# Mario5Gray/Stable-Diffusion-1.5-LCM-ONNX-RKNN2

Hardware: AMD Instinct MI355X
Metric: 512x512 4-step LCM images/sec (higher is better)
Workload: dtype f16; 1 GPU; SD1.5 LCM 512x512, 4 steps, guidance 1.0 (no CFG), batch 1 per GPU, fp16 (fp32 accumulate), hipGraph replay; seeded synthetic SD1.5-architecture weights; batch_per_gpu=1, global_batch=1, image=512x512, lcm_steps=4, parallelism=independent requests x1 (RCCL broadcast of prompt embeddings only)

## Files before the change

include/lcm_hip.h:

```cpp
#ifndef LCM_HIP_H
#define LCM_HIP_H
#include <stdint.h>
#ifdef __cplusplus
extern "C" {
#endif

#define LCM_OK 0
#define LCM_EINVAL (-1)
#define LCM_ENODEV (-2)
#define LCM_EUNSUPPORTED (-3)

#define LCM_EPI_NONE 0
#define LCM_EPI_GEGLU 1
#define LCM_EPI_QUICK_GELU 2
#define LCM_EPI_GELU 3

const char* lcm_last_error(void);
int lcm_version(void);
int lcm_device_info(int dev, char* arch_buf, int buf_len, int* cu_count, uint64_t* hbm_bytes);

int lcm_gemm_f16(const void* A, int lda, const void* A2, int lda2, int K1,
                 const void* W, const void* bias, const void* rowadd, int ld_rowadd, int rows_per_batch,
                 const void* res, int ldr, void* out, int ldo,
                 int M, int N, int K, int epilogue, float out_scale,
                 int batch, int64_t strideA, int64_t strideW, int64_t strideO, int img_rows,
                 void* stats_out, int64_t stats_bytes, int* slabs_per_image, void* stream);
int64_t lcm_stats_bytes(int M, int N, int img_rows);

int lcm_set_workspace(void* ptr, int64_t bytes);
int lcm_set_stream_workspace(void* stream, void* ptr, int64_t bytes);
int lcm_stream_create(void** stream_out);
int lcm_stream_destroy(void* stream);

int lcm_set_tuning(int target_wgs, int max_splits, int min_wgs);
int lcm_set_split_policy(int max_rows_per_image, int max_parts);
int lcm_set_seg_mode(int mode);

int lcm_plan_set(int kind, int M, int N, int K, int aux, int bm, int bn, int splits, int variant);
int lcm_plan_clear(void);
int lcm_canonical_splits(int kind, int m_img, int N, int K, int aux, int ph);

int lcm_gemm_ln_f16(const void* A, int lda, const void* W, const void* ln_g, const void* ln_c, float eps,
                    void* out, int ldo, int M, int N, int K, int epilogue, int img_rows, void* stream);

int lcm_mlp_geglu_f16(const void* x, int ldx, const void* W1, const void* ln_g, const void* ln_c, float eps,
                      const void* W2, const void* b2, void* out, int ldo, int M, int C, int img_rows, void* stream);
int lcm_ln_fold_refresh(const void* W, int N, int K, const void* c_base, const void* c_delta, float alpha,
                        void* g_out, void* c_out, void* stream);

int lcm_set_persist_n(int on);

int lcm_set_kernel_variant(int variant);

int lcm_gemm_tile_config(int M, int N, int batch);

int lcm_conv3x3_f16(const void* in, const void* W, const void* bias,
                    const void* rowadd, int ld_rowadd, const void* res, void* out,
                    int B, int Hin, int Win, int Cin, int Cout, int stride, int ups,
                    void* stats_out, int64_t stats_bytes, int* slabs_per_image, void* stream);

int lcm_conv3x3_down_f16(const void* in, const void* W, const void* bias, void* out, int B, int Hin, int Win, int Cin, int Cout,
                         void* stats_out, int64_t stats_bytes, int* slabs_per_image, void* stream);

int lcm_conv3x3_gn_f16(const void* in, int C1, const void* in2, int C2, const void* gn_scale, const void* gn_shift,
                       int silu, const void* W, const void* bias, const void* rowadd, int ld_rowadd, const void* res,
                       void* out, int B, int Hin, int Win, int Cout, int ups, void* stats_out, int64_t stats_bytes,
                       int* slabs_per_image, void* stream);
int lcm_groupnorm_affine_f16(const void* x, int C1, const void* x2, int C2, const void* gamma, const void* beta,
                             void* scale_out, void* shift_out, int B, int HW, int groups, float eps, void* ws,
                             void* stream);
int lcm_set_halo_pipe_threshold(int wgs);
int lcm_set_halo_prefetch(int on);
int lcm_set_staged_epilogue(int on);
int lcm_set_conv_impl(int impl);

int lcm_conv3x3_c4_f32in(const void* in, const void* pre_w, const void* pre_b, float in_scale,
                         const void* W, const void* bias, void* out, int B, int H, int Wd, int Cout, void* stream);

int lcm_conv3x3_c4_res_f32in(const void* in, const void* W, const void* bias, const void* res, void* out, int B, int H,
                             int Wd, int Cout, void* stream);

int lcm_hint_conv_u8(const void* in, const void* W, const void* bias, void* out, int B, int H, int Wd, int Cout, int silu,
                     void* stream);
int lcm_hint_conv_f16(const void* in, const void* W, const void* bias, void* out, int B, int H, int Wd, int Cin, int Cout,
                      int stride, int silu, void* stream);

int lcm_conv3x3_smalln(const void* in, const void* W, const void* bias, void* out, void* out_f32,
                       int B, int H, int Wd, int Cin, int Cout, int mode, void* stream);
int lcm_conv3x3_smalln_gn(const void* in, const void* gn_scale, const void* gn_shift, int silu, const void* W,
                          const void* bias, void* out, void* out_f32, int B, int H, int Wd, int Cin, int Cout,
                          int mode, void* stream);

int64_t lcm_groupnorm_ws_bytes(int B, int HW, int C, int groups);
int lcm_groupnorm_f16(const void* x, int C1, const void* x2, int C2, const void* gamma, const void* beta,
                      void* out, int B, int HW, int groups, float eps, int silu, void* ws, void* stream);

int lcm_set_gn_fused_bytes(int64_t bytes);
int lcm_groupnorm_from_stats_f16(const void* x, int C1, const void* x2, int C2, const void* stats1, int P1,
                                 const void* stats2, int P2, const void* gamma, const void* beta, void* out,
                                 int B, int HW, int groups, float eps, int silu, void* ws, void* stream);

int lcm_layernorm_f16(const void* x, const void* gamma, const void* beta, void* out, int M, int C, float eps,
                      void* stream);

int lcm_attention_f16(const void* Q, int ldq, const void* K, int ldk, const void* V, int ldv, void* out, int ldo,
                      int B, int heads, int Sq, int Sk, int d, float scale, int causal, void* stream);
int lcm_set_attention_waves(int waves);
int lcm_set_attention_impl(int impl);
int lcm_set_attention_ksplit(int on);

int lcm_embed_tokens_f16(const void* ids, const void* tok_emb, const void* pos_emb, void* out, int B, int S, int D,
                         int vocab, void* stream);

int lcm_prompt_emphasis_f16(const void* z, const void* w, void* out, int ldo, int n_chunks, int S, int D, void* stream);

int lcm_softmax_rows_f16(void* x, int rows, int n, int ld, void* stream);
int lcm_transpose_f16(const void* in, int ldi, void* out, int ldo, int R, int C, int batch,
                      int64_t stride_in, int64_t stride_out, void* stream);

int lcm_linear_smallm_f16(const void* x, int ldx, const void* W, const void* bias, const void* res, int ldr,
                          void* out, int ldo, int M, int N, int K, int silu_in, int silu_out, void* stream);
int lcm_linear_rows_f16(const void* x, int ldx, int x_rows, const void* W, const void* bias, const void* res, int ldr,
                        int res_rows, void* out, int ldo, int M, int N, int K, int silu_in, int silu_out, void* stream);

int lcm_timestep_embedding(float t, void* out, int B, int dim, void* stream);
int lcm_timestep_embedding_steps(const float* t_host, int nsteps, void* out, int B, int dim, void* stream);

int lcm_scheduler_step(const void* eps, const void* eps_uncond, float guidance, void* lat, const void* noise,
                       const float* coef6, int last, int B, int h, int w, void* stream);

#define LCM_PRED_EPSILON 0
#define LCM_PRED_V 1
#define LCM_PRED_SAMPLE 2
int lcm_scheduler_step_ex(const void* eps, const void* eps_uncond, float guidance, void* lat, const void* noise,
                          const float* coef6, int last, int prediction_type, int B, int h, int w, void* stream);

int lcm_latents_renoise(const void* x0, const void* noise, float sqrt_a, float sqrt_b, void* lat_out, int B, int h, int w,
                        int dup, void* stream);
int lcm_scheduler_step_handover(const void* eps, const void* eps_uncond, float guidance, void* lat, const void* noise, void* xk,
                                const float* coef6, float next_sqrt_a, float next_sqrt_b, int prediction_type, int B, int h, int w,
                                int dup, void* stream);

#define LCM_UPSCALE_BILINEAR 0
#define LCM_UPSCALE_BICUBIC 1
#define LCM_UPSCALE_NEAREST_EXACT 2
int lcm_latents_upscale_renoise(const void* x0, int h, int w, const void* noise, float sqrt_a, float sqrt_b, int mode, void* x_up,
                                void* lat_out, int B, int H, int W, int dup, void* stream);

int lcm_vae_enc_conv_in_u8(const void* in, const void* W, const void* bias, void* out, int B, int H, int Wd, int Cout, void* stream);
int lcm_vae_posterior_renoise(const void* pre_mean, const void* pre_logvar, const void* quant_w, const void* quant_b,
                              const void* e0, const void* e1, float scaling_factor, float sqrt_a, float sqrt_b, void* z_out,
                              void* lat_out, void* moments_out, int B, int h, int w, int dup, void* stream);

int lcm_inpaint_mask_prepare(const void* mask_u8, const void* weights_u32, int radius, void* alpha_u8_out, void* scratch_u8,
                             void* latmask_out, int B, int H, int W, void* stream);
int lcm_scheduler_step_inpaint(const void* eps, const void* eps_uncond, float guidance, void* lat, const void* noise, const void* z,
                               const void* e1, const void* latmask, const float* coef6, int last, float next_sqrt_a,
                               float next_sqrt_b, int prediction_type, int B, int h, int w, int dup, void* stream);
int lcm_inpaint_composite_rgb8(void* rgb_inout, const void* init_u8, const void* alpha_u8, int B, int H, int W, void* stream);

long long lcm_canny_ws_bytes(int B, int H, int W);
int lcm_canny_classes_u8(const void* in_rgb, void* cls_out, int B, int H, int W, int lo, int hi, void* stream);
int lcm_canny_link(const void* cls, void* out_rgb, void* ws, long long ws_bytes, int B, int H, int W, void* stream);
int lcm_canny_rgb8(const void* in_rgb, void* out_rgb, void* ws, long long ws_bytes, int B, int H, int W, float low, float high,
                   void* stream);
int lcm_invert_u8(const void* in, void* out, long long n, void* stream);

typedef struct lcm_variation_desc {
    const void* low;
    const void* high;
    int hs, ws;
    float t;
    int active;
} lcm_variation_desc;
#define LCM_VARIATION_MAX_BATCH 8
int lcm_noise_variation_f32(void* lat0, int B, int h, int w, const lcm_variation_desc* descs, void* stream);

int lcm_resize_ksize(int in, int out);
long long lcm_resize_table_bytes(int in, int out, int n);
int lcm_resize_tables(int in, int out, int o0, int n, void* host_dst, long long dst_bytes);
int lcm_resize_span(int in, int out, int o0, int n, int* first, int* last);
int lcm_resize_max_span(int in, int out, int o0, int n, int tile);
int lcm_resize_passes(int sw, int sh, int out_w, int out_h);
long long lcm_resize_plan_table_bytes(int sw, int sh, int out_w, int out_h, int w, int h);
int lcm_resize_plan_tables(int sw, int sh, int out_w, int out_h, int x0, int y0, int w, int h, void* host_dst, long long dst_bytes);
long long lcm_resize_ws_bytes(int C, int sw, int sh, int out_w, int out_h, int x0, int y0, int w, int h);
int lcm_resize_lanczos_u8(const void* src, long long src_stride, int C, int sw, int sh, int out_w, int out_h, int x0, int y0, int w,
                          int h, void* dst, long long dst_stride, void* ws, long long ws_bytes, void* stream);

int lcm_latents_pool8(const void* lat, void* out_f16, int B, int h, int w, void* stream);

int lcm_profile_begin(int max_launches);
int lcm_profile_end(char* out, int64_t cap);
int lcm_debug_spin(int usec, void* stream);
int lcm_debug_grid_barrier(int workgroups, int n_barriers, void* state, void* stream);

long long lcm_png_bound(int width, int height, int stripes);
int lcm_png_encode_rgb8(const void* rgb, int width, int height, long long pitch, int stripes, void* out, long long out_cap,
                        long long* out_len);

int lcm_vae_blend_f32(const void* a, int ah, int aw, void* b, int bh, int bw, int B, int extent, int vertical, void* stream);
int lcm_vae_place_tile(const void* tile, int th, int tw, void* out_u8, void* out_f32, int H, int W, int B,
                       int oy, int ox, int ch, int cw, void* stream);

int lcm_axpy_f16(const void* base, const void* delta, float alpha, void* out, int64_t n, void* stream);

int lcm_sr_conv1(const void* rgb, int W, int H, int tile_w, int tile_h, int t0, int ntiles, const void* w1, const void* b1,
                 void* out, void* stream);
int lcm_sr_conv3x3(const void* in, int T, int th, int tw, int cout, const void* w, const void* bias, void* out, void* stream);
int lcm_sr_conv4_shuffle(const void* in, int W, int H, int tile_w, int tile_h, int t0, int ntiles, const void* w4,
                         const void* b4, int r, void* y_out, void* stream);
int lcm_sr_chroma_h(const void* rgb, int W, int H, int r, void* cbcr_h, void* stream);
int lcm_sr_merge(const void* y_plane, const void* cbcr_h, int W, int H, int r, void* rgb_out, void* stream);

long long lcm_jpeg_coef_bytes(int W, int H);
long long lcm_jpeg_bound(int W, int H);
int lcm_jpeg_quant_tables(int quality, uint8_t* out);
int lcm_jpeg_dct_rgb8(const void* rgb, int W, int H, long long pitch, int quality, void* coefs, long long coefs_bytes,
                      void* stream);
int lcm_jpeg_encode_coefs(const void* coefs, int W, int H, int quality, int threads, void* out, long long out_cap,
                          long long* out_len);

typedef struct lcm_jpeg_info {
    int width, height;
    int ncomp;
    int sampling;
    int restart_interval;
    int mcus_x, mcus_y;
    int blocks_per_mcu;
    long long coefs_bytes;
    long long work_bytes;
    uint8_t qt[3][64];
} lcm_jpeg_info;
int lcm_jpeg_dec_info(const void* data, long long len, lcm_jpeg_info* info);
int lcm_jpeg_dec_coefs(const void* data, long long len, int threads, void* coefs, long long coefs_bytes);
int lcm_jpeg_idct_rgb8(const void* coefs, long long coefs_bytes, const lcm_jpeg_info* info, void* work, long long work_bytes,
                       void* rgb_out, long long pitch, void* stream);

int lcm_graph_begin(void* stream);
int lcm_graph_end(void* stream, void** graph_exec_out);
int lcm_graph_launch(void* graph_exec, void* stream);
int lcm_graph_destroy(void* graph_exec);

#ifdef __cplusplus
}
#endif
#endif
```

stable-diffusion-1.5-lcm-onnx-rknn2_amd/lib.py:

```python
from __future__ import annotations

import ctypes as C
import os
import subprocess

_HERE = os.path.dirname(os.path.abspath(__file__))
LIB_PATH = os.path.join(_HERE, "liblcmhip.so")


class LcmHipError(RuntimeError):
    pass


def build(verbose: bool = False) -> str:
    r = subprocess.run(["make", "-C", os.path.join(_HERE, "csrc"), "-j8"], capture_output=True, text=True)
    if verbose or r.returncode != 0:
        print(r.stdout[-4000:], r.stderr[-4000:])
    if r.returncode != 0:
        raise LcmHipError("building liblcmhip.so failed")
    return LIB_PATH


_vp, _i, _f, _i64 = C.c_void_p, C.c_int, C.c_float, C.c_int64


class VariationDesc(C.Structure):
    _fields_ = [("low", _vp), ("high", _vp), ("hs", _i), ("ws", _i), ("t", _f), ("active", _i)]


VARIATION_MAX_BATCH = 8

_SIGS = {
    "lcm_gemm_f16": [_vp, _i, _vp, _i, _i, _vp, _vp, _vp, _i, _i, _vp, _i, _vp, _i, _i, _i, _i, _i, _f, _i,
                     _i64, _i64, _i64, _i, _vp, _i64, C.POINTER(_i), _vp],
    "lcm_gemm_ln_f16": [_vp, _i, _vp, _vp, _vp, _f, _vp, _i, _i, _i, _i, _i, _i, _vp],
    "lcm_mlp_geglu_f16": [_vp, _i, _vp, _vp, _vp, _f, _vp, _vp, _vp, _i, _i, _i, _i, _vp],
    "lcm_ln_fold_refresh": [_vp, _i, _i, _vp, _vp, _f, _vp, _vp, _vp],
    "lcm_conv3x3_f16": [_vp, _vp, _vp, _vp, _i, _vp, _vp, _i, _i, _i, _i, _i, _i, _i, _vp, _i64, C.POINTER(_i), _vp],
    "lcm_groupnorm_from_stats_f16": [_vp, _i, _vp, _i, _vp, _i, _vp, _i, _vp, _vp, _vp, _i, _i, _i, _f, _i, _vp, _vp],
    "lcm_conv3x3_c4_f32in": [_vp, _vp, _vp, _f, _vp, _vp, _vp, _i, _i, _i, _i, _vp],
    "lcm_conv3x3_c4_res_f32in": [_vp, _vp, _vp, _vp, _vp, _i, _i, _i, _i, _vp],
    "lcm_hint_conv_u8": [_vp, _vp, _vp, _vp, _i, _i, _i, _i, _i, _vp],
    "lcm_hint_conv_f16": [_vp, _vp, _vp, _vp, _i, _i, _i, _i, _i, _i, _i, _vp],
    "lcm_conv3x3_smalln": [_vp, _vp, _vp, _vp, _vp, _i, _i, _i, _i, _i, _i, _vp],
    "lcm_conv3x3_smalln_gn": [_vp, _vp, _vp, _i, _vp, _vp, _vp, _vp, _i, _i, _i, _i, _i, _i, _vp],
    "lcm_groupnorm_f16": [_vp, _i, _vp, _i, _vp, _vp, _vp, _i, _i, _i, _f, _i, _vp, _vp],
    "lcm_layernorm_f16": [_vp, _vp, _vp, _vp, _i, _i, _f, _vp],
    "lcm_attention_f16": [_vp, _i, _vp, _i, _vp, _i, _vp, _i, _i, _i, _i, _i, _i, _f, _i, _vp],
    "lcm_embed_tokens_f16": [_vp, _vp, _vp, _vp, _i, _i, _i, _i, _vp],
    "lcm_prompt_emphasis_f16": [_vp, _vp, _vp, _i, _i, _i, _i, _vp],
    "lcm_softmax_rows_f16": [_vp, _i, _i, _i, _vp],
    "lcm_transpose_f16": [_vp, _i, _vp, _i, _i, _i, _i, _i64, _i64, _vp],
    "lcm_linear_smallm_f16": [_vp, _i, _vp, _vp, _vp, _i, _vp, _i, _i, _i, _i, _i, _i, _vp],
    "lcm_timestep_embedding": [_f, _vp, _i, _i, _vp],
    "lcm_linear_rows_f16": [_vp, _i, _i, _vp, _vp, _vp, _i, _i, _vp, _i, _i, _i, _i, _i, _i, _vp],
    "lcm_timestep_embedding_steps": [_vp, _i, _vp, _i, _i, _vp],
    "lcm_scheduler_step": [_vp, _vp, _f, _vp, _vp, C.POINTER(C.c_float), _i, _i, _i, _i, _vp],
    "lcm_scheduler_step_ex": [_vp, _vp, _f, _vp, _vp, C.POINTER(C.c_float), _i, _i, _i, _i, _i, _vp],
    "lcm_latents_pool8": [_vp, _vp, _i, _i, _i, _vp],
    "lcm_latents_renoise": [_vp, _vp, _f, _f, _vp, _i, _i, _i, _i, _vp],
    "lcm_latents_upscale_renoise": [_vp, _i, _i, _vp, _f, _f, _i, _vp, _vp, _i, _i, _i, _i, _vp],
    "lcm_conv3x3_down_f16": [_vp, _vp, _vp, _vp, _i, _i, _i, _i, _i, _vp, _i64, C.POINTER(_i), _vp],
    "lcm_vae_enc_conv_in_u8": [_vp, _vp, _vp, _vp, _i, _i, _i, _i, _vp],
    "lcm_vae_posterior_renoise": [_vp, _vp, _vp, _vp, _vp, _vp, _f, _f, _f, _vp, _vp, _vp, _i, _i, _i, _i, _vp],
    "lcm_scheduler_step_handover": [_vp, _vp, _f, _vp, _vp, _vp, C.POINTER(C.c_float), _f, _f, _i, _i, _i, _i, _i, _vp],
    "lcm_inpaint_mask_prepare": [_vp, _vp, _i, _vp, _vp, _vp, _i, _i, _i, _vp],
    "lcm_scheduler_step_inpaint": [_vp, _vp, _f, _vp, _vp, _vp, _vp, _vp, C.POINTER(C.c_float), _i, _f, _f, _i, _i, _i, _i, _i, _vp],
    "lcm_inpaint_composite_rgb8": [_vp, _vp, _vp, _i, _i, _i, _vp],
    "lcm_canny_classes_u8": [_vp, _vp, _i, _i, _i, _i, _i, _vp],
    "lcm_canny_link": [_vp, _vp, _vp, C.c_longlong, _i, _i, _i, _vp],
    "lcm_canny_rgb8": [_vp, _vp, _vp, C.c_longlong, _i, _i, _i, _f, _f, _vp],
    "lcm_invert_u8": [_vp, _vp, C.c_longlong, _vp],
    "lcm_noise_variation_f32": [_vp, _i, _i, _i, C.POINTER(VariationDesc), _vp],
    "lcm_resize_lanczos_u8": [_vp, C.c_longlong, _i, _i, _i, _i, _i, _i, _i, _i, _i, _vp, C.c_longlong, _vp, C.c_longlong, _vp],
    "lcm_resize_tables": [_i, _i, _i, _i, _vp, C.c_longlong],
    "lcm_resize_plan_tables": [_i] * 8 + [_vp, C.c_longlong],
    "lcm_resize_span": [_i, _i, _i, _i, C.POINTER(_i), C.POINTER(_i)],
    "lcm_resize_ksize": [_i, _i],
    "lcm_resize_passes": [_i, _i, _i, _i],
    "lcm_resize_max_span": [_i, _i, _i, _i, _i],
    "lcm_png_encode_rgb8": [_vp, _i, _i, C.c_longlong, _i, _vp, C.c_longlong, C.POINTER(C.c_longlong)],
    "lcm_stream_create": [C.POINTER(_vp)],
    "lcm_stream_destroy": [_vp],
    "lcm_graph_begin": [_vp],
    "lcm_graph_end": [_vp, C.POINTER(_vp)],
    "lcm_graph_launch": [_vp, _vp],
    "lcm_graph_destroy": [_vp],
    "lcm_gemm_tile_config": [_i, _i, _i],
    "lcm_debug_spin": [_i, _vp],
    "lcm_debug_grid_barrier": [_i, _i, _vp, _vp],
    "lcm_axpy_f16": [_vp, _vp, _f, _vp, _i64, _vp],
    "lcm_vae_blend_f32": [_vp, _i, _i, _vp, _i, _i, _i, _i, _i, _vp],
    "lcm_vae_place_tile": [_vp, _i, _i, _vp, _vp, _i, _i, _i, _i, _i, _i, _i, _vp],
    "lcm_profile_begin": [_i],
    "lcm_profile_end": [C.c_char_p, _i64],
    "lcm_set_workspace": [_vp, _i64],
    "lcm_set_stream_workspace": [_vp, _vp, _i64],
    "lcm_set_tuning": [_i, _i, _i],
    "lcm_set_split_policy": [_i, _i],
    "lcm_set_seg_mode": [_i],
    "lcm_set_attention_waves": [_i],
    "lcm_set_attention_impl": [_i],
    "lcm_set_attention_ksplit": [_i],
    "lcm_set_kernel_variant": [_i],
    "lcm_set_conv_impl": [_i],
    "lcm_set_persist_n": [_i],
    "lcm_set_halo_pipe_threshold": [_i],
    "lcm_set_halo_prefetch": [_i],
    "lcm_set_staged_epilogue": [_i],
    "lcm_set_gn_fused_bytes": [_i64],
    "lcm_plan_set": [_i] * 9,
    "lcm_plan_clear": [],
    "lcm_canonical_splits": [_i] * 6,
    "lcm_conv3x3_gn_f16": [_vp, _i, _vp, _i, _vp, _vp, _i, _vp, _vp, _vp, _i, _vp, _vp, _i, _i, _i, _i, _i, _vp, _i64,
                           C.POINTER(_i), _vp],
    "lcm_groupnorm_affine_f16": [_vp, _i, _vp, _i, _vp, _vp, _vp, _vp, _i, _i, _i, _f, _vp, _vp],
    "lcm_device_info": [_i, C.c_char_p, _i, C.POINTER(_i), C.POINTER(C.c_uint64)],
    "lcm_sr_conv1": [_vp, _i, _i, _i, _i, _i, _i, _vp, _vp, _vp, _vp],
    "lcm_sr_conv3x3": [_vp, _i, _i, _i, _i, _vp, _vp, _vp, _vp],
    "lcm_sr_conv4_shuffle": [_vp, _i, _i, _i, _i, _i, _i, _vp, _vp, _i, _vp, _vp],
    "lcm_sr_chroma_h": [_vp, _i, _i, _i, _vp, _vp],
    "lcm_sr_merge": [_vp, _vp, _i, _i, _i, _vp, _vp],
    "lcm_jpeg_quant_tables": [_i, _vp],
    "lcm_jpeg_dct_rgb8": [_vp, _i, _i, C.c_longlong, _i, _vp, C.c_longlong, _vp],
    "lcm_jpeg_encode_coefs": [_vp, _i, _i, _i, _i, _vp, C.c_longlong, C.POINTER(C.c_longlong)],
    "lcm_jpeg_dec_info": [_vp, C.c_longlong, _vp],
    "lcm_jpeg_dec_coefs": [_vp, C.c_longlong, _i, _vp, C.c_longlong],
    "lcm_jpeg_idct_rgb8": [_vp, C.c_longlong, _vp, _vp, C.c_longlong, _vp, C.c_longlong, _vp],
}
EXPORTS = tuple(sorted(list(_SIGS) + ["lcm_last_error", "lcm_version", "lcm_groupnorm_ws_bytes", "lcm_stats_bytes", "lcm_png_bound",
                              "lcm_canny_ws_bytes", "lcm_jpeg_coef_bytes", "lcm_jpeg_bound", "lcm_resize_ws_bytes",
                              "lcm_resize_table_bytes", "lcm_resize_plan_table_bytes"]))

EUNSUPPORTED = -3


class JpegInfo(C.Structure):
    _fields_ = [("width", _i), ("height", _i), ("ncomp", _i), ("sampling", _i), ("restart_interval", _i), ("mcus_x", _i),
                ("mcus_y", _i), ("blocks_per_mcu", _i), ("coefs_bytes", C.c_longlong), ("work_bytes", C.c_longlong),
                ("qt", C.c_uint8 * 192)]


_lib = None


def load():
    global _lib
    if _lib is not None:
        return _lib
    if not os.path.exists(LIB_PATH):
        raise LcmHipError(f"{LIB_PATH} not built: run __graft_entry__.build() (make -C csrc); "
                          "there is no CPU fallback for the HIP path")
    import torch
    lib = C.CDLL(LIB_PATH)
    for name, sig in _SIGS.items():
        fn = getattr(lib, name)
        fn.argtypes = sig
        fn.restype = _i
    lib.lcm_last_error.restype = C.c_char_p
    lib.lcm_last_error.argtypes = []
    lib.lcm_version.restype = _i
    lib.lcm_groupnorm_ws_bytes.restype = _i64
    lib.lcm_groupnorm_ws_bytes.argtypes = [_i, _i, _i, _i]
    lib.lcm_stats_bytes.restype = _i64
    lib.lcm_png_bound.restype = C.c_longlong
    lib.lcm_png_bound.argtypes = [_i, _i, _i]
    lib.lcm_stats_bytes.argtypes = [_i, _i, _i]
    lib.lcm_canny_ws_bytes.restype = C.c_longlong
    lib.lcm_canny_ws_bytes.argtypes = [_i, _i, _i]
    for fn, n in ((lib.lcm_resize_ws_bytes, 9), (lib.lcm_resize_table_bytes, 3), (lib.lcm_resize_plan_table_bytes, 6)):
        fn.restype = C.c_longlong
        fn.argtypes = [_i] * n
    for fn in (lib.lcm_jpeg_coef_bytes, lib.lcm_jpeg_bound):
        fn.restype = C.c_longlong
        fn.argtypes = [_i, _i]
    _install_plans(lib)
    _lib = lib
    return lib


PACKAGED_PLANS = os.path.join(_HERE, "tuned_plans_gfx950.json")


def read_plans(path) -> dict:
    import json
    try:
        with open(path) as f:
            return {tuple(int(v) for v in k.split(",")): tuple(val) for k, val in json.load(f).items()}
    except Exception:
        return {}


def known_plans() -> dict:
    plans = {}
    if os.environ.get("LCM_TUNED_PLANS", "1") != "0" and os.path.exists(PACKAGED_PLANS):
        plans.update(read_plans(PACKAGED_PLANS))
    p = os.environ.get("LCM_TUNE_CACHE", "")
    if p and os.path.exists(p):
        plans.update(read_plans(p))
    return plans


def _install_plans(lib):
    for (kind, M, N, K, aux), val in known_plans().items():
        bm, bn, sp, v = (int(x) for x in val[:4])
        lib.lcm_plan_set(kind, M, N, K, aux, bm, bn, sp, v)


def check(rc: int, what: str = ""):
    if rc != 0:
        msg = load().lcm_last_error().decode("utf-8", "replace")
        raise LcmHipError(f"{what or 'lcm call'} failed (rc={rc}): {msg}")


LCM_PRED_EPSILON, LCM_PRED_V, LCM_PRED_SAMPLE = 0, 1, 2
PREDICTION_TYPES = {"epsilon": LCM_PRED_EPSILON, "v_prediction": LCM_PRED_V, "sample": LCM_PRED_SAMPLE}

LCM_UPSCALE_BILINEAR, LCM_UPSCALE_BICUBIC, LCM_UPSCALE_NEAREST_EXACT = 0, 1, 2
UPSCALE_MODES = {"Latent": LCM_UPSCALE_BILINEAR, "Latent (bicubic)": LCM_UPSCALE_BICUBIC,
                 "Latent (nearest-exact)": LCM_UPSCALE_NEAREST_EXACT}
```

stable-diffusion-1.5-lcm-onnx-rknn2_amd/model.py:

```python
from __future__ import annotations

import torch

from . import ops
from .config import TEXT_SEQ_LEN, depth_at, heads_at, unet_config, vae_config
from .packing import pack_conv1x1, pack_conv3x3, pack_conv3x3_up2, pack_ff2_cols, pack_geglu


import os

VAE_FLASH_ATTN = os.environ.get("LCM_VAE_FLASH_ATTN", "1") != "0"
FUSE_GN_MIN_BYTES = int(os.environ.get("LCM_FUSE_GN_MIN_BYTES", str(64 << 20)))


def _fuse_gn_into_conv(M, Cin, Cout):
    if Cin % 64 or Cout % 64:
        return False
    ntiles = Cout // 160 if Cout % 160 == 0 else -(-Cout // 128)
    return M * Cin * 2 >= FUSE_GN_MIN_BYTES and ntiles <= (4 if Cout % 160 == 0 else 3)


class _Buffers:
    def __init__(self, device):
        self.device = device
        self._b = {}

    def get(self, role, *shape, dtype=torch.float16, zero=False):
        key = (role, shape, dtype)
        t = self._b.get(key)
        if t is None:
            t = (torch.zeros if zero else torch.empty)(shape, dtype=dtype, device=self.device)
            self._b[key] = t
        return t

    def nbytes(self):
        return sum(t.numel() * t.element_size() for t in self._b.values())


def _dev(t, device, dtype=torch.float16):
    return t.to(device=device, dtype=dtype).contiguous()


class _Net:
    def __init__(self, device):
        self.device = device
        self.w = {}
        self.buf = _Buffers(device)
        self._stats = {}

    def _put(self, name, t, dtype=torch.float16):
        self.w[name] = _dev(t, self.device, dtype)

    def view(self):
        v = object.__new__(type(self))
        v.__dict__.update(self.__dict__)
        v.buf = _Buffers(self.device)
        v._stats = {}
        return v

    def stats(self, role, M, C, hw):
        key = ("stats", role, M, C, hw)
        st = self._stats.get(key)
        if st is None:
            st = ops.Stats(torch.zeros(ops.stats_floats(M, C, hw), dtype=torch.float32, device=self.device))
            self._stats[key] = st
        return st

    def norm(self, x, gamma, beta, out, B, HW, C1, *, x_st=None, x2=None, C2=0, x2_st=None, eps=1e-5, silu=True):
        C = C1 + C2
        ws = self.gn_ws(B, HW, C)
        if x_st is not None and x_st.P > 0 and (x2 is None or (x2_st is not None and x2_st.P > 0)):
            ops.groupnorm_from_stats(x, gamma, beta, out, B, HW, C1, x_st, ws, x2=x2, C2=C2, st2=x2_st, eps=eps, silu=silu)
        else:
            ops.groupnorm(x, gamma, beta, out, B, HW, C1, ws, x2=x2, C2=C2, eps=eps, silu=silu)
        return out

    def _norm_conv_out(self, x, norm, st, hn, out, B, H, W, ch, cout, eps, *, mode, out_f32=None):
        wt = self.w
        if st is not None and st.P > 0 and ch % 64 == 0:
            sc_t, sh_t = ops.groupnorm_tables_from_stats(wt[norm + ".g"], wt[norm + ".b"], B, H * W, ch, st, self.gn_ws(B, H * W, ch), eps=eps)
            ops.conv3x3_smalln(x, wt["conv_out.w"], out, B, H, W, ch, cout, bias=wt["conv_out.b"], mode=mode, out_f32=out_f32,
                               gn_scale=sc_t, gn_shift=sh_t, silu=True)
        else:
            self.norm(x, wt[norm + ".g"], wt[norm + ".b"], hn, B, H * W, ch, x_st=st, eps=eps)
            ops.conv3x3_smalln(hn, wt["conv_out.w"], out, B, H, W, ch, cout, bias=wt["conv_out.b"], mode=mode, out_f32=out_f32)

    def gn_ws(self, B, HW, C):
        key = ("gn_ws", B, HW, C)
        t = self._stats.get(key)
        if t is None:
            t = torch.empty(max(ops.groupnorm_ws_bytes(B, HW, C) // 4, 1024), dtype=torch.float32, device=self.device)
            self._stats[key] = t
        return t

    def weight_bytes(self):
        return sum(t.numel() * t.element_size() for t in self.w.values())

    def _pack_resnet(self, sd, p, temb_list=None):
        for n in ("norm1", "norm2"):
            self._put(f"{p}.{n}.g", sd[f"{p}.{n}.weight"])
            self._put(f"{p}.{n}.b", sd[f"{p}.{n}.bias"])
        for n in ("conv1", "conv2"):
            self._put(f"{p}.{n}.w", pack_conv3x3(sd[f"{p}.{n}.weight"]))
            self._put(f"{p}.{n}.b", sd[f"{p}.{n}.bias"])
        if f"{p}.conv_shortcut.weight" in sd:
            self._put(f"{p}.sc.w", pack_conv1x1(sd[f"{p}.conv_shortcut.weight"]))
            self._put(f"{p}.sc.b", sd[f"{p}.conv_shortcut.bias"])
        if temb_list is not None:
            temb_list.append((p, sd[f"{p}.time_emb_proj.weight"], sd[f"{p}.time_emb_proj.bias"]))

    def resnet(self, p, x, C1, Cout, B, H, W, eps, x2=None, C2=0, rowadd=None, out_role="res_out", x_st=None, x2_st=None):
        HW, M, Cin = H * W, B * H * W, C1 + C2
        w = self.w
        have1 = x_st is not None and x_st.P > 0 and (x2 is None or (x2_st is not None and x2_st.P > 0))
        sc = x
        if (p + ".sc.w") in w:
            sc = self.buf.get("shortcut", M, Cout)
            ops.gemm(x, w[p + ".sc.w"], sc, bias=w[p + ".sc.b"], a2=x2, img_rows=HW)
        h1 = self.buf.get("conv1", M, Cout)
        h1_st = self.stats("conv1", M, Cout, HW)
        if have1 and C1 % 64 == 0 and C2 % 64 == 0 and _fuse_gn_into_conv(M, Cin, Cout):
            sc_t, sh_t = ops.groupnorm_tables_from_stats(w[p + ".norm1.g"], w[p + ".norm1.b"], B, HW, C1, x_st, self.gn_ws(B, HW, Cin),
                                                         C2=C2, st2=x2_st if x2 is not None else None, eps=eps)
            ops.conv3x3_gn(x, w[p + ".conv1.w"], h1, B, H, W, C1, Cout, x2=x2, C2=C2, gn_scale=sc_t, gn_shift=sh_t, silu=True,
                           bias=w[p + ".conv1.b"], rowadd=rowadd, stats=h1_st)
        else:
            hn = self.buf.get("gn", M, Cin)
            self.norm(x, w[p + ".norm1.g"], w[p + ".norm1.b"], hn, B, HW, C1, x_st=x_st, x2=x2, C2=C2, x2_st=x2_st, eps=eps)
            ops.conv3x3(hn, w[p + ".conv1.w"], h1, B, H, W, Cin, Cout, bias=w[p + ".conv1.b"], rowadd=rowadd, stats=h1_st)
        out = self.buf.get(out_role, M, Cout)
        out_st = self.stats(out_role, M, Cout, HW)
        if h1_st.P > 0 and _fuse_gn_into_conv(M, Cout, Cout):
            sc_t, sh_t = ops.groupnorm_tables_from_stats(w[p + ".norm2.g"], w[p + ".norm2.b"], B, HW, Cout, h1_st,
                                                         self.gn_ws(B, HW, Cout), eps=eps)
            ops.conv3x3_gn(h1, w[p + ".conv2.w"], out, B, H, W, Cout, Cout, gn_scale=sc_t, gn_shift=sh_t, silu=True,
                           bias=w[p + ".conv2.b"], res=sc, stats=out_st)
        else:
            hn2 = self.buf.get("gn", M, Cout)
            self.norm(h1, w[p + ".norm2.g"], w[p + ".norm2.b"], hn2, B, HW, Cout, x_st=h1_st, eps=eps)
            ops.conv3x3(hn2, w[p + ".conv2.w"], out, B, H, W, Cout, Cout, bias=w[p + ".conv2.b"], res=sc, stats=out_st)
        return out, out_st


class _UNetEncoder(_Net):

    def _init_encoder(self, cfg):
        self.cfg = cfg
        boc = cfg["block_out_channels"]
        self.ctx_dim = cfg["cross_attention_dim"]
        self.temb_dim = boc[0] * 4
        self.qs = {}
        self.has_cond = bool(cfg.get("time_cond_proj_dim"))
        self.has_added = bool(cfg.get("addition_time_embed_dim"))

    def _pack_head(self, sd):
        self._put("conv_in.w", pack_conv3x3(sd["conv_in.weight"]))
        self._put("conv_in.b", sd["conv_in.bias"])
        for n in ("linear_1", "linear_2"):
            self._put(f"te.{n}.w", sd[f"time_embedding.{n}.weight"])
            self._put(f"te.{n}.b", sd[f"time_embedding.{n}.bias"])
        if self.has_cond:
            self._put("te.cond.w", sd["time_embedding.cond_proj.weight"])

    def _pack_down_mid(self, sd, temb_list, kv_list):
        cfg = self.cfg
        nb = len(cfg["block_out_channels"])
        for i in range(nb):
            for j in range(cfg["layers_per_block"]):
                self._pack_resnet(sd, f"down_blocks.{i}.resnets.{j}", temb_list)
                if cfg["down_attn"][i]:
                    self._pack_transformer(sd, f"down_blocks.{i}.attentions.{j}", kv_list, depth_at(cfg, i), heads_at(cfg, i))
            if i < nb - 1:
                p = f"down_blocks.{i}.downsamplers.0.conv"
                self._put(p + ".w", pack_conv3x3(sd[p + ".weight"]))
                self._put(p + ".b", sd[p + ".bias"])
        self._pack_resnet(sd, "mid_block.resnets.0", temb_list)
        self._pack_transformer(sd, "mid_block.attentions.0", kv_list, depth_at(cfg, nb - 1), heads_at(cfg, nb - 1))
        self._pack_resnet(sd, "mid_block.resnets.1", temb_list)

    def _pack_tables(self, temb_list, kv_list):
        self.temb_off, off = {}, 0
        for p, wt, bt in temb_list:
            self.temb_off[p] = (off, wt.shape[0])
            off += wt.shape[0]
        self.temb_total = off
        self._put("temb_all.w", torch.cat([t[1] for t in temb_list], 0))
        self._put("temb_all.b", torch.cat([t[2] for t in temb_list], 0))
        self.kv_off, off = {}, 0
        for p, wk, wv in kv_list:
            self.kv_off[p] = (off, wk.shape[0])
            off += 2 * wk.shape[0]
        self.kv_total = off
        self._put("kv_all.w", torch.cat([torch.cat([wk, wv], 0) for _, wk, wv in kv_list], 0))

    def _put_ln_fold(self, name, W, b, gamma, beta, geglu=False):
        Wf, g32, b32 = W.float(), gamma.float(), beta.float()
        Wg = Wf * g32[None, :]
        c = Wf @ b32 + (b.float() if b is not None else 0.0)
        if geglu:
            Wg, c = pack_geglu(Wg, c)
        Wh = Wg.to(torch.float16)
        self._put(name + ".w", Wh)
        self._put(name + ".g", torch.zeros(Wh.shape[0]), torch.float32)
        ops.ln_fold_refresh(self.w[name + ".w"], self.w[name + ".g"])
        self._put(name + ".c", c, torch.float32)
        self._put(name + ".lnw", g32, torch.float32)
        self._put(name + ".lnb", b32, torch.float32)

    def _pack_transformer(self, sd, p, kv_list, depth=1, heads=8):
        self._put(p + ".norm.g", sd[p + ".norm.weight"])
        self._put(p + ".norm.b", sd[p + ".norm.bias"])
        self._put(p + ".proj_in.w", pack_conv1x1(sd[p + ".proj_in.weight"]))
        self._put(p + ".proj_in.b", sd[p + ".proj_in.bias"])
        self._put(p + ".proj_out.w", pack_conv1x1(sd[p + ".proj_out.weight"]))
        self._put(p + ".proj_out.b", sd[p + ".proj_out.bias"])
        for k in range(depth):
            t, q = f"{p}.transformer_blocks.{k}", f"{p}.{k}"
            wqkv = torch.cat([sd[f"{t}.attn1.to_{n}.weight"] for n in "qkv"], 0).float()
            wq2, wff, bff = sd[f"{t}.attn2.to_q.weight"].float(), sd[f"{t}.ff.net.0.proj.weight"], sd[f"{t}.ff.net.0.proj.bias"]
            C = wq2.shape[0]
            self.qs[q] = qs = (C // heads) ** -0.5 * 1.4426950408889634
            wqkv[:C] *= qs
            wq2 = wq2 * qs
            self._put_ln_fold(q + ".qkv", wqkv, None, sd[f"{t}.norm1.weight"], sd[f"{t}.norm1.bias"])
            self._put_ln_fold(q + ".q2", wq2, None, sd[f"{t}.norm2.weight"], sd[f"{t}.norm2.bias"])
            self._put_ln_fold(q + ".ff1", wff, bff, sd[f"{t}.norm3.weight"], sd[f"{t}.norm3.bias"], geglu=True)
            self._put(q + ".o1.w", sd[f"{t}.attn1.to_out.0.weight"])
            self._put(q + ".o1.b", sd[f"{t}.attn1.to_out.0.bias"])
            self._put(q + ".o2.w", sd[f"{t}.attn2.to_out.0.weight"])
            self._put(q + ".o2.b", sd[f"{t}.attn2.to_out.0.bias"])
            kv_list.append((q, sd[f"{t}.attn2.to_k.weight"], sd[f"{t}.attn2.to_v.weight"]))
            self._put(q + ".ff2.w", pack_ff2_cols(sd[f"{t}.ff.net.2.weight"]))
            self._put(q + ".ff2.b", sd[f"{t}.ff.net.2.bias"])

    def encode_context(self, ehs, B):
        Sk = ehs.shape[0] // B
        if Sk * B != ehs.shape[0] or Sk % TEXT_SEQ_LEN:
            raise ValueError(f"encode_context: {ehs.shape[0]} context rows are not {B} x a multiple of {TEXT_SEQ_LEN}")
        kv = self.buf.get("kv_all", B * Sk, self.kv_total)
        ops.gemm(ehs, self.w["kv_all.w"], kv, img_rows=Sk)
        return kv

    def encode_added(self, add_in, B):
        w = self.w
        h = self.buf.get("add_h", B, self.temb_dim)
        ops.linear_smallm(add_in, w["add.linear_1.w"], h, B, self.temb_dim, self.added_dim, bias=w["add.linear_1.b"], silu_out=True)
        aug = self.buf.get("add_aug", B, self.temb_dim)
        ops.linear_smallm(h, w["add.linear_2.w"], aug, B, self.temb_dim, self.temb_dim, bias=w["add.linear_2.b"])
        return aug

    def time_embed(self, t, wemb, B, aug=None):
        w = self.w
        ch0 = self.cfg["block_out_channels"][0]
        e0 = self.buf.get("te0", B, ch0)
        ops.timestep_embedding(float(t), e0, B, ch0)
        if self.has_cond and wemb is not None:
            e1 = self.buf.get("te1", B, ch0)
            ops.linear_smallm(wemb, w["te.cond.w"], e1, B, ch0, wemb.shape[1], res=e0)
        else:
            e1 = e0
        h = self.buf.get("te_h", B, self.temb_dim)
        ops.linear_smallm(e1, w["te.linear_1.w"], h, B, self.temb_dim, ch0, bias=w["te.linear_1.b"], silu_out=True)
        temb = self.buf.get("temb", B, self.temb_dim)
        ops.linear_smallm(h, w["te.linear_2.w"], temb, B, self.temb_dim, self.temb_dim, bias=w["te.linear_2.b"], res=aug, silu_out=True)
        ta = self.buf.get("temb_all", B, self.temb_total)
        self._temb_proj(temb, ta)
        return ta

    MAX_HOISTED_STEPS = 64

    def time_embed_all(self, ts, wemb, B, aug=None):
        w = self.w
        S, ch0 = len(ts), self.cfg["block_out_channels"][0]
        M = S * B
        e0 = self.buf.get("te0_all", M, ch0)
        ops.timestep_embedding_steps([float(t) for t in ts], e0, B, ch0)
        if self.has_cond and wemb is not None:
            e1 = self.buf.get("te1_all", M, ch0)
            ops.linear_rows(wemb, w["te.cond.w"], e1, M, ch0, wemb.shape[1], x_rows=B, res=e0)
        else:
            e1 = e0
        h = self.buf.get("te_h_all", M, self.temb_dim)
        ops.linear_rows(e1, w["te.linear_1.w"], h, M, self.temb_dim, ch0, bias=w["te.linear_1.b"], silu_out=True)
        temb = self.buf.get("temb_rows", M, self.temb_dim)
        ops.linear_rows(h, w["te.linear_2.w"], temb, M, self.temb_dim, self.temb_dim, bias=w["te.linear_2.b"], res=aug, res_rows=B,
                        silu_out=True)
        ta = self.buf.get("temb_all_rows", M, self.temb_total)
        self._temb_proj(temb, ta)
        return ta

    def _temb_proj(self, temb, ta):
        w = self.w
        ops.gemm(temb, w["temb_all.w"], ta, bias=w["temb_all.b"], img_rows=1)

    def _res(self, p, x, C1, Cout, B, H, W, ta, x2=None, C2=0, out_role="res_out", x_st=None, x2_st=None):
        off, n = self.temb_off[p]
        return self.resnet(p, x, C1, Cout, B, H, W, self.cfg["norm_eps"], x2=x2, C2=C2, rowadd=ta[:, off:off + n],
                           out_role=out_role, x_st=x_st, x2_st=x2_st)

    def transformer(self, p, x, C, B, H, W, kv_all, out_role, x_st=None, heads=8, depth=1):
        w = self.w
        HW, M, d = H * W, B * H * W, C // heads
        Sk = kv_all.shape[0] // B
        hn = self.buf.get("gn", M, C)
        self.norm(x, w[p + ".norm.g"], w[p + ".norm.b"], hn, B, HW, C, x_st=x_st, eps=1e-6, silu=False)
        h = self.buf.get("tf_h", M, C)
        ops.gemm(hn, w[p + ".proj_in.w"], h, bias=w[p + ".proj_in.b"], img_rows=HW)
        qkv = self.buf.get("tf_qkv", M, 3 * C)
        a = self.buf.get("tf_attn", M, C)
        q2 = self.buf.get("tf_q2", M, C)
        ff = self.buf.get("tf_ff", M, 4 * C)
        for k in range(depth):
            q = f"{p}.{k}"
            ops.gemm_ln(h, w[q + ".qkv.w"], w[q + ".qkv.g"], w[q + ".qkv.c"], qkv, img_rows=HW)
            ops.attention(qkv[:, :C], qkv[:, C:2 * C], qkv[:, 2 * C:], a, B, heads, HW, HW, d, ldq=3 * C, ldk=3 * C,
                          ldv=3 * C, ldo=C, scale=0.0)
            ops.gemm(a, w[q + ".o1.w"], h, bias=w[q + ".o1.b"], res=h, img_rows=HW)
            ops.gemm_ln(h, w[q + ".q2.w"], w[q + ".q2.g"], w[q + ".q2.c"], q2, img_rows=HW)
            off, _ = self.kv_off[q]
            ops.attention(q2, kv_all[:, off:off + C], kv_all[:, off + C:off + 2 * C], a, B, heads, HW, Sk, d,
                          ldq=C, ldk=self.kv_total, ldv=self.kv_total, ldo=C, scale=0.0)
            ops.gemm(a, w[q + ".o2.w"], h, bias=w[q + ".o2.b"], res=h, img_rows=HW)
            if ops.mlp_fused_applies(M, C, HW):
                ops.mlp_geglu(h, w[q + ".ff1.w"], w[q + ".ff1.g"], w[q + ".ff1.c"], w[q + ".ff2.w"], w[q + ".ff2.b"], h, img_rows=HW)
                continue
            ops.gemm_ln(h, w[q + ".ff1.w"], w[q + ".ff1.g"], w[q + ".ff1.c"], ff, epilogue=1, img_rows=HW)
            ops.gemm(ff, w[q + ".ff2.w"], h, bias=w[q + ".ff2.b"], res=h, img_rows=HW)
        out = self.buf.get(out_role, M, C)
        out_st = self.stats(out_role, M, C, HW)
        ops.gemm(h, w[p + ".proj_out.w"], out, bias=w[p + ".proj_out.b"], res=x, stats=out_st, img_rows=HW)
        return out, out_st

    def _down_mid(self, x, B, H, W, kv_all, ta, tap):
        cfg, wt = self.cfg, self.w
        boc = cfg["block_out_channels"]
        nb = len(boc)
        skips = [(x, boc[0], None)]
        ch, ns, st = boc[0], 1, None
        sizes = [(H, W)]
        for i in range(nb):
            for j in range(cfg["layers_per_block"]):
                p = f"down_blocks.{i}.resnets.{j}"
                attn = cfg["down_attn"][i]
                x, st = self._res(p, x, ch, boc[i], B, H, W, ta, out_role="res_out" if attn else f"skip{ns}", x_st=st)
                ch = boc[i]
                tap(p, x, ch, H, W)
                if attn:
                    p = f"down_blocks.{i}.attentions.{j}"
                    x, st = self.transformer(p, x, ch, B, H, W, kv_all, f"skip{ns}", x_st=st, heads=heads_at(cfg, i),
                                             depth=depth_at(cfg, i))
                    tap(p, x, ch, H, W)
                skips.append((x, ch, st))
                ns += 1
            if i < nb - 1:
                p = f"down_blocks.{i}.downsamplers.0.conv"
                H2, W2 = (H + 1) // 2, (W + 1) // 2
                y = self.buf.get(f"skip{ns}", B * H2 * W2, ch)
                st = self.stats(f"skip{ns}", B * H2 * W2, ch, H2 * W2)
                ops.conv3x3(x, wt[p + ".w"], y, B, H, W, ch, ch, bias=wt[p + ".b"], stride=2, stats=st)
                H, W, x = H2, W2, y
                sizes.append((H, W))
                skips.append((x, ch, st))
                ns += 1
        x, st = self._res("mid_block.resnets.0", x, ch, ch, B, H, W, ta, x_st=st)
        x, st = self.transformer("mid_block.attentions.0", x, ch, B, H, W, kv_all, "tf_out", x_st=st,
                                 heads=heads_at(cfg, nb - 1), depth=depth_at(cfg, nb - 1))
        x, st = self._res("mid_block.resnets.1", x, ch, ch, B, H, W, ta, out_role="cur", x_st=st)
        tap("mid_block.resnets.1", x, ch, H, W)
        return x, st, skips, sizes, ch, H, W


class UNetHip(_UNetEncoder):
    def __init__(self, sd: dict, cfg: dict | None = None, device="cuda"):
        super().__init__(device)
        cfg = unet_config(cfg)
        self._init_encoder(cfg)
        boc = cfg["block_out_channels"]
        nb = len(boc)
        temb_list, kv_list = [], []
        self._pack_head(sd)
        if self.has_added:
            for n in ("linear_1", "linear_2"):
                self._put(f"add.{n}.w", sd[f"add_embedding.{n}.weight"])
                self._put(f"add.{n}.b", sd[f"add_embedding.{n}.bias"])
            self.added_dim = cfg["projection_class_embeddings_input_dim"]
        self._pack_down_mid(sd, temb_list, kv_list)
        up_attn = tuple(reversed(cfg["down_attn"]))
        for i in range(nb):
            for j in range(cfg["layers_per_block"] + 1):
                self._pack_resnet(sd, f"up_blocks.{i}.resnets.{j}", temb_list)
                if up_attn[i]:
                    self._pack_transformer(sd, f"up_blocks.{i}.attentions.{j}", kv_list, depth_at(cfg, nb - 1 - i), heads_at(cfg, nb - 1 - i))
            if i < nb - 1:
                p = f"up_blocks.{i}.upsamplers.0.conv"
                self._put(p + ".w", pack_conv3x3_up2(sd[p + ".weight"]))
                self._put(p + ".w3", pack_conv3x3(sd[p + ".weight"]))
                self._put(p + ".b", sd[p + ".bias"])
        self._put("conv_norm_out.g", sd["conv_norm_out.weight"])
        self._put("conv_norm_out.b", sd["conv_norm_out.bias"])
        self._put("conv_out.w", pack_conv3x3(sd["conv_out.weight"]))
        self._put("conv_out.b", sd["conv_out.bias"])
        self._pack_tables(temb_list, kv_list)

    def forward(self, lat, t, kv_all, wemb, B, h, w_, eps_out, taps=None, aug=None, ta=None, control=None):
        cfg, wt = self.cfg, self.w
        boc = cfg["block_out_channels"]
        nb = len(boc)
        if ta is None:
            ta = self.time_embed(t, wemb, B, aug)
        H, W = h, w_
        x = self.buf.get("skip0", B * H * W, boc[0])
        ops.conv3x3_c4(lat, wt["conv_in.w"], x, B, H, W, boc[0], bias=wt["conv_in.b"])

        def tap(name, t_, C, H_, W_):
            if taps is not None:
                taps[name] = t_.reshape(B, H_, W_, C).permute(0, 3, 1, 2).float().cpu()

        tap("conv_in", x, boc[0], H, W)
        x, st, skips, sizes, ch, H, W = self._down_mid(x, B, H, W, kv_all, ta, tap)
        if control is not None:
            cn, feats, mid_f, cscale = control
            lv, k = [], 0
            for i in range(nb):
                lv += [i] * (cfg["layers_per_block"] + (1 if i == 0 else 0))
                if i < nb - 1:
                    lv.append(i + 1)
            for k, (s, sc, _) in enumerate(skips):
                Hs, Ws = sizes[lv[k]]
                o = self.buf.get(f"ctl_skip{k}", s.shape[0], sc)
                cn.inject(k, feats[k][0], s, o, cscale, Hs * Ws, B, Hs, Ws, taps)
                skips[k] = (o, sc, None)
                tap(f"ctl.skip.{k}", o, sc, Hs, Ws)
            o = self.buf.get("ctl_mid", x.shape[0], ch)
            cn.inject("mid", mid_f, x, o, cscale, H * W, B, H, W, taps)
            x, st = o, None
            tap("ctl.mid", x, ch, H, W)
        rboc = tuple(reversed(boc))
        up_attn = tuple(reversed(cfg["down_attn"]))
        for i in range(nb):
            for j in range(cfg["layers_per_block"] + 1):
                s, sc, s_st = skips.pop()
                p = f"up_blocks.{i}.resnets.{j}"
                x, st = self._res(p, x, ch, rboc[i], B, H, W, ta, x2=s, C2=sc, out_role="res_out" if up_attn[i] else "cur",
                                  x_st=st, x2_st=s_st)
                ch = rboc[i]
                tap(p, x, ch, H, W)
                if up_attn[i]:
                    p = f"up_blocks.{i}.attentions.{j}"
                    x, st = self.transformer(p, x, ch, B, H, W, kv_all, "cur", x_st=st, heads=heads_at(cfg, nb - 1 - i),
                                             depth=depth_at(cfg, nb - 1 - i))
                    tap(p, x, ch, H, W)
            if i < nb - 1:
                p = f"up_blocks.{i}.upsamplers.0.conv"
                Ho, Wo = sizes[nb - 2 - i]
                y = self.buf.get("ups", B * Ho * Wo, ch)
                st = self.stats("ups", B * Ho * Wo, ch, Ho * Wo)
                if (Ho, Wo) == (2 * H, 2 * W):
                    ops.conv3x3(x, wt[p + ".w"], y, B, H, W, ch, ch, bias=wt[p + ".b"], ups=2, stats=st)
                else:
                    ops.conv3x3(x, wt[p + ".w3"], y, B, H, W, ch, ch, bias=wt[p + ".b"], ups=1, stats=st, out_hw=(Ho, Wo))
                H, W, x = Ho, Wo, y
                tap(f"up_blocks.{i}.upsamplers.0", x, ch, H, W)
        hn = self.buf.get("gn", B * H * W, ch)
        self._norm_conv_out(x, "conv_norm_out", st, hn, eps_out, B, H, W, ch, cfg["out_channels"], cfg["norm_eps"], mode=0)
        return eps_out



class ControlNetHip(_UNetEncoder):

    def __init__(self, sd: dict, cfg: dict | None = None, unet_cfg: dict | None = None, device="cuda"):
        super().__init__(device)
        from .weights import check_controlnet_matches, controlnet_config
        cfg = controlnet_config(unet_cfg) if cfg is None else dict(cfg)
        check_controlnet_matches(cfg, unet_config(unet_cfg))
        cfg = unet_config(cfg)
        cfg["time_cond_proj_dim"] = None
        self._init_encoder(cfg)
        self.cond_channels = cc = tuple(cfg["conditioning_embedding_out_channels"])
        e = "controlnet_cond_embedding"
        names = [e + ".conv_in"] + [f"{e}.blocks.{i}" for i in range(2 * (len(cc) - 1))] + [e + ".conv_out"]
        for i, n in enumerate(names):
            self._put(f"hint.{i}.w", pack_conv3x3(sd[n + ".weight"]))
            self._put(f"hint.{i}.b", sd[n + ".bias"])
        temb_list, kv_list = [], []
        self._pack_head(sd)
        self._pack_down_mid(sd, temb_list, kv_list)
        self._pack_tables(temb_list, kv_list)
        from .weights import controlnet_skip_channels
        self.n_down = len(controlnet_skip_channels(cfg))
        for i in list(range(self.n_down)) + ["mid"]:
            n = f"controlnet_down_blocks.{i}" if i != "mid" else "controlnet_mid_block"
            self._put(f"zero.{i}.w", pack_conv1x1(sd[n + ".weight"]))
            self._put(f"zero.{i}.b", sd[n + ".bias"])

    def embed_hint(self, hint_u8, B, H, W, out):
        w, cc = self.w, self.cond_channels
        x = self.buf.get("hint0", B * H * W, cc[0])
        ops.hint_conv_u8(hint_u8, w["hint.0.w"], x, B, H, W, cc[0], bias=w["hint.0.b"], silu=True)
        for i in range(2 * (len(cc) - 1)):
            cin, cout, stride = cc[i // 2], cc[i // 2 + (i & 1)], 1 + (i & 1)
            Ho, Wo = ((H + 1) // 2, (W + 1) // 2) if stride == 2 else (H, W)
            y = self.buf.get(f"hint{i + 1}", B * Ho * Wo, cout)
            ops.hint_conv(x, w[f"hint.{i + 1}.w"], y, B, H, W, cin, cout, bias=w[f"hint.{i + 1}.b"], stride=stride, silu=True)
            x, H, W = y, Ho, Wo
        n = 2 * len(cc) - 1
        ops.conv3x3(x, w[f"hint.{n}.w"], out, B, H, W, cc[-1], self.cfg["block_out_channels"][0], bias=w[f"hint.{n}.b"])
        return out

    def forward(self, lat, t, kv_all, B, h, w_, hint_emb, taps=None, ta=None):
        boc = self.cfg["block_out_channels"]
        if ta is None:
            ta = self.time_embed(t, None, B)
        x = self.buf.get("skip0", B * h * w_, boc[0])
        ops.conv3x3_c4_res(lat, self.w["conv_in.w"], x, B, h, w_, boc[0], bias=self.w["conv_in.b"], res=hint_emb)

        def tap(name, t_, C, H_, W_):
            if taps is not None:
                taps["cn." + name] = t_.reshape(B, H_, W_, C).permute(0, 3, 1, 2).float().cpu()

        tap("conv_in", x, boc[0], h, w_)
        x, _, skips, _, _, _, _ = self._down_mid(x, B, h, w_, kv_all, ta, tap)
        return skips, x

    def inject(self, i, feat, skip, out, scale, img_rows, B, H, W, taps=None):
        ops.gemm(feat, self.w[f"zero.{i}.w"], out, bias=self.w[f"zero.{i}.b"], res=skip, out_scale=float(scale), img_rows=img_rows)
        if taps is not None:
            C = out.shape[1]
            r = torch.empty_like(out)
            ops.gemm(feat, self.w[f"zero.{i}.w"], r, bias=self.w[f"zero.{i}.b"], out_scale=float(scale), img_rows=img_rows)
            taps[f"ctl.res.{i}"] = r.reshape(B, H, W, C).permute(0, 3, 1, 2).float().cpu()
            taps[f"ctl.feat.{i}"] = feat.reshape(B, H, W, C).permute(0, 3, 1, 2).float().cpu()


def scale_vae_residual_stream(sd: dict, cfg: dict, s: float) -> dict:
    out = dict(sd)

    def mul(name):
        out[name] = (sd[name].float() * s).to(sd[name].dtype)

    for n in ("decoder.conv_in.weight", "decoder.conv_in.bias", "decoder.mid_block.attentions.0.to_out.0.weight",
              "decoder.mid_block.attentions.0.to_out.0.bias"):
        mul(n)
    resnets = ["decoder.mid_block.resnets.0", "decoder.mid_block.resnets.1"]
    nb = len(cfg["block_out_channels"])
    for i in range(nb):
        resnets += [f"decoder.up_blocks.{i}.resnets.{j}" for j in range(cfg["layers_per_block"] + 1)]
        if i < nb - 1:
            mul(f"decoder.up_blocks.{i}.upsamplers.0.conv.bias")
    for r in resnets:
        mul(r + ".conv2.weight")
        mul(r + ".conv2.bias")
        if r + ".conv_shortcut.bias" in sd:
            mul(r + ".conv_shortcut.bias")
    return out


class _VAENet(_Net):

    def _pack_mid_attention(self, sd, a, C):
        self._put("attn.norm.g", sd[a + ".group_norm.weight"])
        self._put("attn.norm.b", sd[a + ".group_norm.bias"])
        self.flash_attn = VAE_FLASH_ATTN and C == 512
        if self.flash_attn:
            self._put("attn.qkv.w", torch.cat([sd[f"{a}.{n}.weight"].reshape(C, C) for n in ("to_q", "to_k", "to_v")], 0))
            self._put("attn.qkv.b", torch.cat([sd[f"{a}.{n}.bias"] for n in ("to_q", "to_k", "to_v")], 0))
        else:
            for n in ("to_q", "to_k", "to_v"):
                self._put(f"attn.{n}.w", sd[f"{a}.{n}.weight"].reshape(C, C))
                self._put(f"attn.{n}.b", sd[f"{a}.{n}.bias"])
        self._put("attn.o.w", sd[a + ".to_out.0.weight"].reshape(C, C))
        self._put("attn.o.b", sd[a + ".to_out.0.bias"])

    def mid_attention(self, x, C, B, H, W, x_st=None):
        w = self.w
        S, M = H * W, B * H * W
        hn = self.buf.get("gn", M, C)
        self.norm(x, w["attn.norm.g"], w["attn.norm.b"], hn, B, S, C, x_st=x_st, eps=1e-6, silu=False)
        out = self.buf.get("res_out2", M, C)
        out_st = self.stats("res_out2", M, C, S)
        if self.flash_attn:
            qkv = self.buf.get("attn_qkv", M, 3 * C)
            ops.gemm(hn, w["attn.qkv.w"], qkv, bias=w["attn.qkv.b"], img_rows=S)
            o = self.buf.get("attn_o", M, C)
            ops.attention(qkv[:, :C], qkv[:, C:2 * C], qkv[:, 2 * C:], o, B, 1, S, S, C, ldq=3 * C, ldk=3 * C, ldv=3 * C, ldo=C)
            ops.gemm(o, w["attn.o.w"], out, bias=w["attn.o.b"], res=x, stats=out_st, img_rows=S)
            return out, out_st
        Sp = -(-S // 64) * 64
        q, v = self.buf.get("attn_q", M, C), self.buf.get("attn_v", M, C)
        k = self.buf.get("attn_k", B * Sp, C, zero=True)
        ops.gemm(hn, w["attn.to_q.w"], q, bias=w["attn.to_q.b"], img_rows=S)
        ops.gemm(hn, w["attn.to_v.w"], v, bias=w["attn.to_v.b"], img_rows=S)
        if Sp == S:
            ops.gemm(hn, w["attn.to_k.w"], k, bias=w["attn.to_k.b"], img_rows=S)
        else:
            ops.gemm(hn, w["attn.to_k.w"], k, bias=w["attn.to_k.b"], M=S, N=C, K=C, lda=C, ldo=C, batch=B, strideA=S * C,
                     strideW=0, strideO=Sp * C)
        sc = self.buf.get("attn_scores", B * S, Sp)
        ops.gemm(q, k, sc, M=S, N=Sp, K=C, lda=C, ldo=Sp, batch=B, strideA=S * C, strideW=Sp * C, strideO=S * Sp,
                 out_scale=C ** -0.5)
        ops.softmax_rows(sc, B * S, S, Sp)
        vt = self.buf.get("attn_vt", B * C, Sp, zero=True)
        ops.transpose(v, vt, S, C, ldi=C, ldo=Sp, batch=B, stride_in=S * C, stride_out=C * Sp)
        o = self.buf.get("attn_o", M, C)
        ops.gemm(sc, vt, o, M=S, N=C, K=Sp, lda=Sp, ldo=C, batch=B, strideA=S * Sp, strideW=C * Sp, strideO=S * C)
        ops.gemm(o, w["attn.o.w"], out, bias=w["attn.o.b"], res=x, stats=out_st, img_rows=S)
        return out, out_st


class VAEDecoderHip(_VAENet):
    def __init__(self, sd: dict, cfg: dict | None = None, device="cuda"):
        super().__init__(device)
        self.cfg = cfg = vae_config(cfg)
        boc = cfg["block_out_channels"]
        if float(cfg.get("residual_scale", 1.0)) != 1.0:
            sd = scale_vae_residual_stream(sd, cfg, float(cfg["residual_scale"]))
        self._put("pq.w", sd["post_quant_conv.weight"].reshape(4, 4), torch.float32)
        self._put("pq.b", sd["post_quant_conv.bias"], torch.float32)
        self._put("conv_in.w", pack_conv3x3(sd["decoder.conv_in.weight"]))
        self._put("conv_in.b", sd["decoder.conv_in.bias"])
        self._pack_resnet(sd, "decoder.mid_block.resnets.0")
        self._pack_resnet(sd, "decoder.mid_block.resnets.1")
        self._pack_mid_attention(sd, "decoder.mid_block.attentions.0", boc[-1])
        nb = len(boc)
        for i in range(nb):
            for j in range(cfg["layers_per_block"] + 1):
                self._pack_resnet(sd, f"decoder.up_blocks.{i}.resnets.{j}")
            if i < nb - 1:
                p = f"decoder.up_blocks.{i}.upsamplers.0.conv"
                self._put(p + ".w", pack_conv3x3_up2(sd[p + ".weight"]))
                self._put(p + ".b", sd[p + ".bias"])
        self._put("norm_out.g", sd["decoder.conv_norm_out.weight"])
        self._put("norm_out.b", sd["decoder.conv_norm_out.bias"])
        self._put("conv_out.w", pack_conv3x3(sd["decoder.conv_out.weight"]))
        self._put("conv_out.b", sd["decoder.conv_out.bias"])

    def decode(self, lat, B, h, w_, rgb_out, img_f32=None, taps=None, use_tiling=True):
        tmin = int(self.cfg.get("sample_size", 512)) // 8
        if use_tiling and (h > tmin or w_ > tmin):
            return self.decode_tiled(lat, B, h, w_, rgb_out, img_f32)
        return self.decode_plain(lat, B, h, w_, rgb_out, img_f32, taps)

    def decode_tiled(self, lat, B, h, w_, rgb_out, img_f32=None, overlap=0.25):
        sample = int(self.cfg.get("sample_size", 512))
        tl = sample // 8
        stride, extent = int(tl * (1 - overlap)), int(sample * overlap)
        limit = sample - extent
        H, W = 8 * h, 8 * w_
        ys, xs = list(range(0, h, stride)), list(range(0, w_, stride))
        tiles = {}
        for i, y0 in enumerate(ys):
            for j, x0 in enumerate(xs):
                th, tw = min(tl, h - y0), min(tl, w_ - x0)
                sub = self.buf.get("tile_lat", B, 4, th, tw, dtype=torch.float32)
                sub.copy_(lat[:, :, y0:y0 + th, x0:x0 + tw])
                img = self.buf.get(f"tile_img_{i}_{j}", B, 8 * th, 8 * tw, 3, dtype=torch.float32)
                scratch = self.buf.get("tile_u8", B, 8 * th, 8 * tw, 3, dtype=torch.uint8)
                self.decode_plain(sub, B, th, tw, scratch, img_f32=img)
                tiles[(i, j)] = (img, 8 * th, 8 * tw)
        oy = 0
        for i in range(len(ys)):
            ox = 0
            for j in range(len(xs)):
                img, th, tw = tiles[(i, j)]
                if i > 0:
                    a, ah, aw = tiles[(i - 1, j)]
                    ops.vae_blend(a, ah, aw, img, th, tw, B, min(ah, th, extent), True)
                if j > 0:
                    a, ah, aw = tiles[(i, j - 1)]
                    ops.vae_blend(a, ah, aw, img, th, tw, B, min(aw, tw, extent), False)
                ch, cw = min(limit, th), min(limit, tw)
                ops.vae_place_tile(img, th, tw, rgb_out, img_f32, H, W, B, oy, ox, ch, cw)
                ox += cw
            oy += min(limit, tiles[(i, 0)][1])
        return rgb_out

    def decode_plain(self, lat, B, h, w_, rgb_out, img_f32=None, taps=None):
        cfg, wt = self.cfg, self.w
        boc = cfg["block_out_channels"]
        H, W = h, w_
        ch = boc[-1]

        def tap(name, t_, C, H_, W_):
            if taps is not None:
                taps[name] = t_.reshape(B, H_, W_, C).permute(0, 3, 1, 2).float().cpu()

        x = self.buf.get("cur", B * H * W, ch)
        ops.conv3x3_c4(lat, wt["conv_in.w"], x, B, H, W, ch, bias=wt["conv_in.b"], pre_w=wt["pq.w"], pre_b=wt["pq.b"],
                       in_scale=1.0 / cfg["scaling_factor"])
        tap("decoder.conv_in", x, ch, H, W)
        x, st = self.resnet("decoder.mid_block.resnets.0", x, ch, ch, B, H, W, 1e-6)
        tap("decoder.mid_block.resnets.0", x, ch, H, W)
        x, st = self.mid_attention(x, ch, B, H, W, x_st=st)
        tap("decoder.mid_block.attentions.0", x, ch, H, W)
        x, st = self.resnet("decoder.mid_block.resnets.1", x, ch, ch, B, H, W, 1e-6, out_role="cur", x_st=st)
        rboc = tuple(reversed(boc))
        nb = len(boc)
        roles = ("res_out", "cur")
        for i in range(nb):
            for j in range(cfg["layers_per_block"] + 1):
                p = f"decoder.up_blocks.{i}.resnets.{j}"
                x, st = self.resnet(p, x, ch, rboc[i], B, H, W, 1e-6, out_role=roles[j & 1], x_st=st)
                ch = rboc[i]
                tap(p, x, ch, H, W)
            if i < nb - 1:
                p = f"decoder.up_blocks.{i}.upsamplers.0.conv"
                y = self.buf.get("ups", B * 4 * H * W, ch)
                st = self.stats("ups", B * 4 * H * W, ch, 4 * H * W)
                ops.conv3x3(x, wt[p + ".w"], y, B, H, W, ch, ch, bias=wt[p + ".b"], ups=2, stats=st)
                H, W, x = 2 * H, 2 * W, y
                tap(f"decoder.up_blocks.{i}.upsamplers.0", x, ch, H, W)
        hn = self.buf.get("gn", B * H * W, ch)
        self._norm_conv_out(x, "norm_out", st, hn, rgb_out, B, H, W, ch, cfg["out_channels"], 1e-6, mode=1, out_f32=img_f32)
        return rgb_out


class VAEEncoderHip(_VAENet):

    def __init__(self, sd: dict, cfg: dict | None = None, device="cuda"):
        super().__init__(device)
        self.cfg = cfg = vae_config(cfg)
        boc = cfg["block_out_channels"]
        if float(cfg.get("residual_scale", 1.0)) != 1.0:
            raise ValueError("VAEEncoderHip: a VAE that needs residual scaling (force_upcast, the SDXL family) is not served")
        if "encoder.conv_in.weight" not in sd or "quant_conv.weight" not in sd:
            raise KeyError("this checkpoint carries no AutoencoderKL encoder (encoder.* / quant_conv.* tensors)")
        lc = cfg["latent_channels"]
        if lc != 4:
            raise ValueError(f"VAEEncoderHip: latent_channels {lc} (the posterior launch is written for 4)")
        self._put("conv_in.w", pack_conv3x3(sd["encoder.conv_in.weight"]))
        self._put("conv_in.b", sd["encoder.conv_in.bias"])
        nb = len(boc)
        for i in range(nb):
            for j in range(cfg["layers_per_block"]):
                self._pack_resnet(sd, f"encoder.down_blocks.{i}.resnets.{j}")
            if i < nb - 1:
                p = f"encoder.down_blocks.{i}.downsamplers.0.conv"
                self._put(p + ".w", pack_conv3x3(sd[p + ".weight"]))
                self._put(p + ".b", sd[p + ".bias"])
        self._pack_resnet(sd, "encoder.mid_block.resnets.0")
        self._pack_resnet(sd, "encoder.mid_block.resnets.1")
        self._pack_mid_attention(sd, "encoder.mid_block.attentions.0", boc[-1])
        self._put("norm_out.g", sd["encoder.conv_norm_out.weight"])
        self._put("norm_out.b", sd["encoder.conv_norm_out.bias"])
        wo, bo = sd["encoder.conv_out.weight"], sd["encoder.conv_out.bias"]
        for n, r in (("mean", slice(0, lc)), ("logvar", slice(lc, 2 * lc))):
            self._put(f"conv_out.{n}.w", pack_conv3x3(wo[r]))
            self._put(f"conv_out.{n}.b", bo[r])
        self._put("quant.w", sd["quant_conv.weight"].reshape(2 * lc, 2 * lc), torch.float32)
        self._put("quant.b", sd["quant_conv.bias"], torch.float32)

    def mid_block(self, x, ch, B, H, W, x_st=None):
        x, st = self.resnet("encoder.mid_block.resnets.0", x, ch, ch, B, H, W, 1e-6, x_st=x_st)
        x, st = self.mid_attention(x, ch, B, H, W, x_st=st)
        return self.resnet("encoder.mid_block.resnets.1", x, ch, ch, B, H, W, 1e-6, out_role="cur", x_st=st)

    def encode(self, img_u8, B, H, W, taps=None):
        cfg, wt = self.cfg, self.w
        boc = cfg["block_out_channels"]
        nb = len(boc)

        def tap(name, t_, C, H_, W_):
            if taps is not None:
                taps[name] = t_.reshape(B, H_, W_, C).permute(0, 3, 1, 2).float().cpu()

        ch = boc[0]
        x = self.buf.get("enc_in", B * H * W, ch)
        ops.vae_enc_conv_in_u8(img_u8, wt["conv_in.w"], x, B, H, W, ch, bias=wt["conv_in.b"])
        tap("encoder.conv_in", x, ch, H, W)
        st = None
        roles = ("res_out", "cur")
        for i in range(nb):
            for j in range(cfg["layers_per_block"]):
                p = f"encoder.down_blocks.{i}.resnets.{j}"
                x, st = self.resnet(p, x, ch, boc[i], B, H, W, 1e-6, out_role=roles[j & 1], x_st=st)
                ch = boc[i]
                tap(p, x, ch, H, W)
            if i < nb - 1:
                p = f"encoder.down_blocks.{i}.downsamplers.0.conv"
                Ho, Wo = (H - 2) // 2 + 1, (W - 2) // 2 + 1
                y = self.buf.get("down", B * Ho * Wo, ch)
                st = self.stats("down", B * Ho * Wo, ch, Ho * Wo)
                ops.conv3x3_down(x, wt[p + ".w"], y, B, H, W, ch, ch, bias=wt[p + ".b"], stats=st)
                H, W, x = Ho, Wo, y
                tap(f"encoder.down_blocks.{i}.downsamplers.0", x, ch, H, W)
        x, st = self.mid_block(x, ch, B, H, W, x_st=st)
        tap("encoder.mid_block", x, ch, H, W)
        pre_m = self.buf.get("pre_mean", B, H, W, 4, dtype=torch.float32)
        pre_l = self.buf.get("pre_logvar", B, H, W, 4, dtype=torch.float32)
        if st is not None and st.P > 0 and ch % 64 == 0:
            sc_t, sh_t = ops.groupnorm_tables_from_stats(wt["norm_out.g"], wt["norm_out.b"], B, H * W, ch, st, self.gn_ws(B, H * W, ch), eps=1e-6)
            for n, o in (("mean", pre_m), ("logvar", pre_l)):
                ops.conv3x3_smalln(x, wt[f"conv_out.{n}.w"], o, B, H, W, ch, 4, bias=wt[f"conv_out.{n}.b"], mode=0,
                                   gn_scale=sc_t, gn_shift=sh_t, silu=True)
        else:
            hn = self.buf.get("gn", B * H * W, ch)
            self.norm(x, wt["norm_out.g"], wt["norm_out.b"], hn, B, H * W, ch, x_st=st, eps=1e-6)
            for n, o in (("mean", pre_m), ("logvar", pre_l)):
                ops.conv3x3_smalln(hn, wt[f"conv_out.{n}.w"], o, B, H, W, ch, 4, bias=wt[f"conv_out.{n}.b"], mode=0)
        return pre_m, pre_l, H, W
```

stable-diffusion-1.5-lcm-onnx-rknn2_amd/ops.py:

```python
from __future__ import annotations

import ctypes as C

import torch

from . import lib as _lib


def _p(t):
    return None if t is None else C.c_void_p(t.data_ptr())


def _stream():
    return C.c_void_p(torch.cuda.current_stream().cuda_stream)


import contextlib
import functools
import threading

_hooks = threading.local()


def _record_list():
    return getattr(_hooks, "record", None)


def _profile_list():
    return getattr(_hooks, "profile", None)


@contextlib.contextmanager
def recording():
    prev, recs = _record_list(), []
    _hooks.record = recs
    try:
        yield recs
    finally:
        _hooks.record = prev


@contextlib.contextmanager
def profiling():
    prev, recs = _profile_list(), []
    _hooks.profile = recs
    try:
        yield recs
    finally:
        _hooks.profile = prev


class _Timed:

    def __init__(self, kind, flops, bytes_):
        self.rec = None
        if _profile_list() is not None:
            self.rec = dict(kind=kind, flops=float(flops), bytes=float(bytes_))

    def __enter__(self):
        return self

    def __exit__(self, *a):
        if self.rec is not None:
            pl = _profile_list()
            if pl is not None:
                pl.append(self.rec)
        return False


def plan_set(kind, M, N, K, aux, bm, bn, splits, variant=-1):
    _lib.check(_lib.load().lcm_plan_set(kind, M, N, K, aux, bm, bn, splits, variant), "lcm_plan_set")


def plan_clear():
    _lib.check(_lib.load().lcm_plan_clear(), "lcm_plan_clear")


def plan_reset():
    plan_clear()
    _lib._install_plans(_lib.load())


def canonical_splits(kind, m_img, N, K, aux=1, ph=0):
    n = _lib.load().lcm_canonical_splits(int(kind), int(m_img), int(N), int(K), int(aux), int(ph))
    if n < 0:
        _lib.check(n, "lcm_canonical_splits")
    return n


class Stats:

    __slots__ = ("buf", "P")

    def __init__(self, buf):
        self.buf = buf
        self.P = 0


def stats_floats(M, N, hw=None):
    return int(_lib.load().lcm_stats_bytes(int(M), int(N), int(hw) if hw else 0)) // 4


def _stats_args(stats):
    if stats is None:
        return None, 0, None
    sp = C.c_int(0)
    return _p(stats.buf), stats.buf.numel() * stats.buf.element_size(), sp


def gemm(a, w, out, *, bias=None, res=None, rowadd=None, rows_per_batch=0, a2=None, epilogue=0, out_scale=1.0,
         M=None, N=None, K=None, lda=None, ldo=None, batch=1, strideA=0, strideW=0, strideO=0, stats=None, img_rows=0):
    L = _lib.load()
    sbuf, sbytes, sp = _stats_args(stats)
    M = a.shape[0] if M is None else M
    K1 = a.shape[-1] if a2 is not None else 0
    K = (a.shape[-1] + (a2.shape[-1] if a2 is not None else 0)) if K is None else K
    N = w.shape[0] if N is None else N
    lda = a.stride(-2) if lda is None else lda
    ldo = out.stride(-2) if ldo is None else ldo
    RECORD = _record_list()
    if RECORD is not None:
        kw = dict(bias=bias, res=res, rowadd=rowadd, rows_per_batch=rows_per_batch, a2=a2, epilogue=epilogue,
                  out_scale=out_scale, M=M, N=N, K=K, lda=lda, ldo=ldo, batch=batch, strideA=strideA, strideW=strideW,
                  strideO=strideO, stats=stats, img_rows=img_rows)
        RECORD.append(((0, M, N, K, batch), dict(halo=False, geglu=(epilogue == 1), m_img=(img_rows if img_rows and M % img_rows == 0 else M),
                                                 splittable=(epilogue == 0 and batch == 1 and not (strideA or strideW or strideO))),
                       lambda: gemm(a, w, out, **kw)))
    with _Timed("gemm", 2.0 * M * N * K * batch, 2.0 * batch * (M * K + N * K + M * N)):
        rc = L.lcm_gemm_f16(_p(a), lda, _p(a2), a2.stride(0) if a2 is not None else 0, K1, _p(w), _p(bias), _p(rowadd),
                            rowadd.stride(0) if rowadd is not None else 0, rows_per_batch,
                            _p(res), res.stride(0) if res is not None else 0, _p(out), ldo,
                            M, N, K, epilogue, float(out_scale), batch, strideA, strideW, strideO, int(img_rows),
                            sbuf, sbytes, C.byref(sp) if sp is not None else None, _stream())
    if stats is not None:
        stats.P = sp.value
    _lib.check(rc, "lcm_gemm_f16")
    return out


def gemm_ln(a, w, ln_g, ln_c, out, *, eps=1e-5, epilogue=0, img_rows=0):
    L = _lib.load()
    M, K = a.shape
    N = w.shape[0]
    RECORD = _record_list()
    if RECORD is not None:
        RECORD.append(((0, M, N, K, 1), dict(halo=False, geglu=(epilogue == 1), m_img=(img_rows if img_rows and M % img_rows == 0 else M),
                                             splittable=False),
                       lambda: gemm_ln(a, w, ln_g, ln_c, out, eps=eps, epilogue=epilogue, img_rows=img_rows)))
    with _Timed("gemm", 2.0 * M * N * K, 2.0 * (M * K + N * K + M * N)):
        rc = L.lcm_gemm_ln_f16(_p(a), a.stride(0), _p(w), _p(ln_g), _p(ln_c), float(eps), _p(out), out.stride(0), M, N, K,
                               int(epilogue), int(img_rows), _stream())
    _lib.check(rc, "lcm_gemm_ln_f16")
    return out


import os as _os

_MLP_FUSED_MIN_ROWS = int(_os.environ.get("LCM_MLP_FUSED_MIN_ROWS", "24576") or 0)


def mlp_fused_applies(M, C, img_rows):
    if _MLP_FUSED_MIN_ROWS <= 0 or C != 320 or M < _MLP_FUSED_MIN_ROWS:
        return False
    m_img = img_rows if img_rows and M % img_rows == 0 else M
    return canonical_splits(0, m_img, C, 4 * C, 1, 0) == 1


def mlp_geglu(x, w1, ln_g, ln_c, w2, b2, out, *, eps=1e-5, img_rows=0):
    L = _lib.load()
    M, Cc = x.shape
    F = w2.shape[1]
    RECORD = _record_list()
    if RECORD is not None:
        RECORD.append((None, None, lambda: mlp_geglu(x, w1, ln_g, ln_c, w2, b2, out, eps=eps, img_rows=img_rows)))
    with _Timed("mlp", 2.0 * M * (2 * F) * Cc + 2.0 * M * Cc * F, 2.0 * (2 * M * Cc + 2 * F * Cc + Cc * F)):
        rc = L.lcm_mlp_geglu_f16(_p(x), x.stride(0), _p(w1), _p(ln_g), _p(ln_c), float(eps), _p(w2), _p(b2), _p(out),
                                 out.stride(0), M, Cc, int(img_rows), _stream())
    _lib.check(rc, "lcm_mlp_geglu_f16")
    return out


def ln_fold_refresh(w, g_out, c_base=None, c_delta=None, alpha=0.0, c_out=None):
    _lib.check(_lib.load().lcm_ln_fold_refresh(_p(w), w.shape[0], w.shape[1], _p(c_base), _p(c_delta), float(alpha), _p(g_out),
                                               _p(c_out), _stream()), "lcm_ln_fold_refresh")


def conv3x3(x, w, out, B, H, W, Cin, Cout, *, bias=None, rowadd=None, res=None, stride=1, ups=0, stats=None, out_hw=None):
    L = _lib.load()
    sbuf, sbytes, sp = _stats_args(stats)
    Ho, Wo = ((2 * H, 2 * W) if ups else ((H + 1) // 2, (W + 1) // 2) if stride == 2 else (H, W))
    flags = ups
    if out_hw is not None and tuple(out_hw) != (Ho, Wo):
        if ups != 1 or out_hw[0] not in (2 * H, 2 * H - 1) or out_hw[1] not in (2 * W, 2 * W - 1):
            raise _lib.LcmHipError(f"conv3x3: output size {tuple(out_hw)} from {H}x{W} needs ups=1 (plain 3x3 weights) and 2n / 2n-1 "
                                   f"targets, got ups={ups}")
        flags = ups | (4 if out_hw[0] == 2 * H - 1 else 0) | (8 if out_hw[1] == 2 * W - 1 else 0)
        Ho, Wo = out_hw
    Mo = B * Ho * Wo
    taps = 4 if ups == 2 else 9
    RECORD = _record_list()
    if RECORD is not None:
        kw = dict(bias=bias, rowadd=rowadd, res=res, stride=stride, ups=ups, stats=stats, out_hw=out_hw)
        key = (1, Mo, Cout, 9 * Cin, 1) if stride == 2 else (2, Mo, Cout, taps * Cin, (Wo << 1))
        RECORD.append((key, dict(halo=stride == 1, W=(W if ups == 2 else Wo), phases=4 if ups == 2 else 1, m_img=Mo // B, splittable=True),
                       lambda: conv3x3(x, w, out, B, H, W, Cin, Cout, **kw)))
    with _Timed("conv3x3", 2.0 * Mo * Cout * taps * Cin, 2.0 * (B * H * W * Cin + 9 * Cin * Cout + Mo * Cout)):
        rc = L.lcm_conv3x3_f16(_p(x), _p(w), _p(bias), _p(rowadd), rowadd.stride(0) if rowadd is not None else 0,
                               _p(res), _p(out), B, H, W, Cin, Cout, stride, flags, sbuf, sbytes,
                               C.byref(sp) if sp is not None else None, _stream())
    if stats is not None:
        stats.P = sp.value
    _lib.check(rc, "lcm_conv3x3_f16")
    return out


def conv3x3_down(x, w, out, B, H, W, Cin, Cout, *, bias=None, stats=None):
    L = _lib.load()
    sbuf, sbytes, sp = _stats_args(stats)
    Ho, Wo = (H - 2) // 2 + 1, (W - 2) // 2 + 1
    Mo = B * Ho * Wo
    RECORD = _record_list()
    if RECORD is not None:
        RECORD.append(((1, Mo, Cout, 9 * Cin, 1), dict(halo=False, W=Wo, phases=1, m_img=Mo // B, splittable=True),
                       lambda: conv3x3_down(x, w, out, B, H, W, Cin, Cout, bias=bias, stats=stats)))
    with _Timed("conv3x3", 2.0 * Mo * Cout * 9 * Cin, 2.0 * (B * H * W * Cin + 9 * Cin * Cout + Mo * Cout)):
        rc = L.lcm_conv3x3_down_f16(_p(x), _p(w), _p(bias), _p(out), B, H, W, Cin, Cout, sbuf, sbytes,
                                    C.byref(sp) if sp is not None else None, _stream())
    if stats is not None:
        stats.P = sp.value
    _lib.check(rc, "lcm_conv3x3_down_f16")
    return out


def conv3x3_gn(x, w, out, B, H, W, C1, Cout, *, x2=None, C2=0, gn_scale=None, gn_shift=None, silu=True, bias=None,
               rowadd=None, res=None, ups=0, stats=None):
    L = _lib.load()
    sbuf, sbytes, sp = _stats_args(stats)
    Cin = C1 + (C2 if x2 is not None else 0)
    Ho, Wo = (2 * H, 2 * W) if ups else (H, W)
    Mo = B * Ho * Wo
    RECORD = _record_list()
    if RECORD is not None:
        kw = dict(x2=x2, C2=C2, gn_scale=gn_scale, gn_shift=gn_shift, silu=silu, bias=bias, rowadd=rowadd, res=res, ups=ups,
                  stats=stats)
        RECORD.append(((2, Mo, Cout, 9 * Cin, (Wo << 1) | (1 if gn_scale is not None else 0)),
                       dict(halo=True, W=Wo, m_img=Mo // B, splittable=True), lambda: conv3x3_gn(x, w, out, B, H, W, C1, Cout, **kw)))
    with _Timed("conv3x3", 2.0 * Mo * Cout * 9 * Cin, 2.0 * (B * H * W * Cin + 9 * Cin * Cout + Mo * Cout)):
        rc = L.lcm_conv3x3_gn_f16(_p(x), C1, _p(x2), C2 if x2 is not None else 0, _p(gn_scale), _p(gn_shift),
                                  1 if silu else 0, _p(w), _p(bias), _p(rowadd),
                                  rowadd.stride(0) if rowadd is not None else 0, _p(res), _p(out), B, H, W, Cout, ups,
                                  sbuf, sbytes, C.byref(sp) if sp is not None else None, _stream())
    if stats is not None:
        stats.P = sp.value
    _lib.check(rc, "lcm_conv3x3_gn_f16")
    return out


def groupnorm_affine(x, gamma, beta, scale, shift, B, HW, C1, ws, *, x2=None, C2=0, groups=32, eps=1e-5):
    L = _lib.load()
    rc = L.lcm_groupnorm_affine_f16(_p(x), C1, _p(x2), C2 if x2 is not None else 0, _p(gamma), _p(beta), _p(scale),
                                    _p(shift), B, HW, groups, float(eps), _p(ws), _stream())
    _lib.check(rc, "lcm_groupnorm_affine_f16")


def set_halo_pipe_threshold(wgs):
    _lib.check(_lib.load().lcm_set_halo_pipe_threshold(int(wgs)), "lcm_set_halo_pipe_threshold")


def set_halo_prefetch(on):
    _lib.check(_lib.load().lcm_set_halo_prefetch(1 if on else 0), "lcm_set_halo_prefetch")


def set_persist_n(on):
    _lib.check(_lib.load().lcm_set_persist_n(1 if on else 0), "lcm_set_persist_n")


def set_conv_impl(impl):
    _lib.check(_lib.load().lcm_set_conv_impl(int(impl)), "lcm_set_conv_impl")


def conv3x3_c4(lat_f32, w, out, B, H, W, Cout, *, bias=None, pre_w=None, pre_b=None, in_scale=1.0):
    L = _lib.load()
    rc = L.lcm_conv3x3_c4_f32in(_p(lat_f32), _p(pre_w), _p(pre_b), float(in_scale), _p(w), _p(bias), _p(out),
                                B, H, W, Cout, _stream())
    _lib.check(rc, "lcm_conv3x3_c4_f32in")
    return out


def conv3x3_c4_res(lat_f32, w, out, B, H, W, Cout, *, bias=None, res):
    L = _lib.load()
    rc = L.lcm_conv3x3_c4_res_f32in(_p(lat_f32), _p(w), _p(bias), _p(res), _p(out), B, H, W, Cout, _stream())
    _lib.check(rc, "lcm_conv3x3_c4_res_f32in")
    return out


def hint_conv_u8(img_u8, w, out, B, H, W, Cout, *, bias=None, silu=True):
    L = _lib.load()
    _lib.check(L.lcm_hint_conv_u8(_p(img_u8), _p(w), _p(bias), _p(out), B, H, W, Cout, 1 if silu else 0, _stream()), "lcm_hint_conv_u8")
    return out


def vae_enc_conv_in_u8(img_u8, w, out, B, H, W, Cout, *, bias=None):
    L = _lib.load()
    _lib.check(L.lcm_vae_enc_conv_in_u8(_p(img_u8), _p(w), _p(bias), _p(out), B, H, W, Cout, _stream()), "lcm_vae_enc_conv_in_u8")
    return out


def vae_posterior_renoise(pre_mean, pre_logvar, quant_w, quant_b, e0, e1, scaling, sqrt_a, sqrt_b, z_out, lat, B, h, w, *,
                          moments=None, dup=False):
    L = _lib.load()
    _lib.check(L.lcm_vae_posterior_renoise(_p(pre_mean), _p(pre_logvar), _p(quant_w), _p(quant_b), _p(e0), _p(e1), float(scaling),
                                           float(sqrt_a), float(sqrt_b), _p(z_out), _p(lat), _p(moments), int(B), int(h), int(w),
                                           int(bool(dup)), _stream()), "lcm_vae_posterior_renoise")
    return lat


def hint_conv(x, w, out, B, H, W, Cin, Cout, *, bias=None, stride=1, silu=True):
    L = _lib.load()
    _lib.check(L.lcm_hint_conv_f16(_p(x), _p(w), _p(bias), _p(out), B, H, W, Cin, Cout, int(stride), 1 if silu else 0, _stream()),
               "lcm_hint_conv_f16")
    return out


def conv3x3_smalln(x, w, out, B, H, W, Cin, Cout, *, bias=None, mode=0, out_f32=None, gn_scale=None, gn_shift=None, silu=True):
    L = _lib.load()
    if gn_scale is not None:
        rc = L.lcm_conv3x3_smalln_gn(_p(x), _p(gn_scale), _p(gn_shift), 1 if silu else 0, _p(w), _p(bias), _p(out), _p(out_f32),
                                     B, H, W, Cin, Cout, mode, _stream())
    else:
        rc = L.lcm_conv3x3_smalln(_p(x), _p(w), _p(bias), _p(out), _p(out_f32), B, H, W, Cin, Cout, mode, _stream())
    _lib.check(rc, "lcm_conv3x3_smalln")
    return out


def groupnorm_ws_bytes(B, HW, C, groups=32):
    return int(_lib.load().lcm_groupnorm_ws_bytes(B, HW, C, groups))


def groupnorm(x, gamma, beta, out, B, HW, C1, ws, *, x2=None, C2=0, groups=32, eps=1e-5, silu=True):
    L = _lib.load()
    rc = L.lcm_groupnorm_f16(_p(x), C1, _p(x2), C2, _p(gamma), _p(beta), _p(out), B, HW, groups, float(eps),
                             1 if silu else 0, _p(ws), _stream())
    _lib.check(rc, "lcm_groupnorm_f16")
    return out


def groupnorm_from_stats(x, gamma, beta, out, B, HW, C1, st1, ws, *, x2=None, C2=0, st2=None, groups=32, eps=1e-5, silu=True):
    L = _lib.load()
    rc = L.lcm_groupnorm_from_stats_f16(_p(x), C1, _p(x2), C2 if x2 is not None else 0, _p(st1.buf), st1.P,
                                        _p(st2.buf) if st2 is not None else None, st2.P if st2 is not None else 0,
                                        _p(gamma), _p(beta), _p(out), B, HW, groups, float(eps), 1 if silu else 0, _p(ws), _stream())
    _lib.check(rc, "lcm_groupnorm_from_stats_f16")
    return out


def groupnorm_tables_from_stats(gamma, beta, B, HW, C1, st1, ws, *, C2=0, st2=None, groups=32, eps=1e-5):
    L = _lib.load()
    C = C1 + (C2 if st2 is not None else 0)
    rc = L.lcm_groupnorm_from_stats_f16(None, C1, None, C2 if st2 is not None else 0, _p(st1.buf), st1.P,
                                        _p(st2.buf) if st2 is not None else None, st2.P if st2 is not None else 0,
                                        _p(gamma), _p(beta), None, B, HW, groups, float(eps), 0, _p(ws), _stream())
    _lib.check(rc, "lcm_groupnorm_from_stats_f16")
    return ws[:B * C].view(B, C), ws[B * C:2 * B * C].view(B, C)


def layernorm(x, gamma, beta, out, M, C, eps=1e-5):
    L = _lib.load()
    _lib.check(L.lcm_layernorm_f16(_p(x), _p(gamma), _p(beta), _p(out), M, C, float(eps), _stream()), "lcm_layernorm_f16")
    return out


def embed_tokens(ids, tok_emb, pos_emb, out, B, S, D):
    L = _lib.load()
    _lib.check(L.lcm_embed_tokens_f16(_p(ids), _p(tok_emb), _p(pos_emb), _p(out), B, S, D, tok_emb.shape[0], _stream()),
               "lcm_embed_tokens_f16")
    return out


def prompt_emphasis(z, w, out, n_chunks, S, D, ldo=None):
    L = _lib.load()
    ldo = out.stride(0) if ldo is None else ldo
    _lib.check(L.lcm_prompt_emphasis_f16(_p(z), _p(w), _p(out), int(ldo), int(n_chunks), int(S), int(D), _stream()),
               "lcm_prompt_emphasis_f16")
    _record_plain(lambda: prompt_emphasis(z, w, out, n_chunks, S, D, ldo))
    return out


def attention(q, k, v, out, B, heads, Sq, Sk, d, *, ldq, ldk, ldv, ldo, scale=None, causal=False):
    L = _lib.load()
    scale = d ** -0.5 if scale is None else scale
    RECORD = _record_list()
    if RECORD is not None:
        RECORD.append((None, None, lambda: attention(q, k, v, out, B, heads, Sq, Sk, d, ldq=ldq, ldk=ldk, ldv=ldv, ldo=ldo,
                                                     scale=scale, causal=causal)))
    with _Timed("attention", 4.0 * B * heads * Sq * Sk * d, 2.0 * B * heads * d * (2 * Sq + 2 * Sk)):
        rc = L.lcm_attention_f16(_p(q), ldq, _p(k), ldk, _p(v), ldv, _p(out), ldo, B, heads, Sq, Sk, d, float(scale),
                                 1 if causal else 0, _stream())
    _lib.check(rc, "lcm_attention_f16")
    return out


def softmax_rows(x, rows, n, ld):
    L = _lib.load()
    _lib.check(L.lcm_softmax_rows_f16(_p(x), rows, n, ld, _stream()), "lcm_softmax_rows_f16")
    return x


def transpose(x, out, R, Cc, *, ldi, ldo, batch=1, stride_in=0, stride_out=0):
    L = _lib.load()
    _lib.check(L.lcm_transpose_f16(_p(x), ldi, _p(out), ldo, R, Cc, batch, stride_in, stride_out, _stream()), "lcm_transpose_f16")
    return out


def linear_smallm(x, w, out, M, N, K, *, bias=None, res=None, silu_in=False, silu_out=False, ldx=None, ldo=None):
    L = _lib.load()
    rc = L.lcm_linear_smallm_f16(_p(x), x.stride(0) if ldx is None else ldx, _p(w), _p(bias), _p(res),
                                 res.stride(0) if res is not None else 0, _p(out), out.stride(0) if ldo is None else ldo,
                                 M, N, K, int(silu_in), int(silu_out), _stream())
    _lib.check(rc, "lcm_linear_smallm_f16")
    return out


def linear_rows(x, w, out, M, N, K, *, x_rows=None, bias=None, res=None, res_rows=None, silu_in=False, silu_out=False):
    L = _lib.load()
    rc = L.lcm_linear_rows_f16(_p(x), x.stride(0), M if x_rows is None else x_rows, _p(w), _p(bias), _p(res),
                               res.stride(0) if res is not None else 0, M if res_rows is None else res_rows, _p(out), out.stride(0),
                               M, N, K, int(silu_in), int(silu_out), _stream())
    _lib.check(rc, "lcm_linear_rows_f16")
    return out


def timestep_embedding_steps(ts, out, B, dim):
    L = _lib.load()
    arr = (C.c_float * len(ts))(*[float(t) for t in ts])
    _lib.check(L.lcm_timestep_embedding_steps(arr, len(ts), _p(out), B, dim, _stream()), "lcm_timestep_embedding_steps")
    return out


def timestep_embedding(t, out, B, dim):
    L = _lib.load()
    _lib.check(L.lcm_timestep_embedding(float(t), _p(out), B, dim, _stream()), "lcm_timestep_embedding")
    return out


def scheduler_step(eps, lat, noise, coef6, last, B, h, w, *, eps_uncond=None, guidance=1.0, pred="epsilon"):
    L = _lib.load()
    arr = (C.c_float * 6)(*[float(c) for c in coef6])
    if pred == "epsilon":
        rc = L.lcm_scheduler_step(_p(eps), _p(eps_uncond), float(guidance), _p(lat), _p(noise), arr, int(bool(last)),
                                  B, h, w, _stream())
        _lib.check(rc, "lcm_scheduler_step")
        return lat
    if pred not in _lib.PREDICTION_TYPES:
        raise ValueError(f"unknown prediction type {pred!r}: expected one of {sorted(_lib.PREDICTION_TYPES)}")
    rc = L.lcm_scheduler_step_ex(_p(eps), _p(eps_uncond), float(guidance), _p(lat), _p(noise), arr, int(bool(last)),
                                 _lib.PREDICTION_TYPES[pred], B, h, w, _stream())
    _lib.check(rc, "lcm_scheduler_step_ex")
    return lat


def latents_renoise(x0, noise, sqrt_a, sqrt_b, lat, B, h, w, *, dup=False):
    L = _lib.load()
    _lib.check(L.lcm_latents_renoise(_p(x0), _p(noise), float(sqrt_a), float(sqrt_b), _p(lat), B, h, w, int(bool(dup)), _stream()),
               "lcm_latents_renoise")
    return lat


def latents_upscale_renoise(x0, h, w, noise, sqrt_a, sqrt_b, mode, lat, B, H, W, *, x_up=None, dup=False):
    L = _lib.load()
    _lib.check(L.lcm_latents_upscale_renoise(_p(x0), int(h), int(w), _p(noise), float(sqrt_a), float(sqrt_b), int(mode), _p(x_up),
                                             _p(lat), int(B), int(H), int(W), int(bool(dup)), _stream()),
               "lcm_latents_upscale_renoise")
    return lat


def scheduler_step_handover(eps, lat, noise, xk, coef6, next_sqrt_a, next_sqrt_b, B, h, w, *, eps_uncond=None, guidance=1.0,
                            pred="epsilon", dup=False):
    if pred not in _lib.PREDICTION_TYPES:
        raise ValueError(f"unknown prediction type {pred!r}: expected one of {sorted(_lib.PREDICTION_TYPES)}")
    L = _lib.load()
    arr = (C.c_float * 6)(*[float(c) for c in coef6])
    rc = L.lcm_scheduler_step_handover(_p(eps), _p(eps_uncond), float(guidance), _p(lat), _p(noise), _p(xk), arr, float(next_sqrt_a),
                                       float(next_sqrt_b), _lib.PREDICTION_TYPES[pred], B, h, w, int(bool(dup)), _stream())
    _lib.check(rc, "lcm_scheduler_step_handover")
    return lat


def _record_plain(replay):
    RECORD = _record_list()
    if RECORD is not None:
        RECORD.append((None, None, replay))


def inpaint_mask_prepare(mask_u8, weights_u32, radius, alpha_out, scratch, latmask_out, B, H, W):
    L = _lib.load()
    _lib.check(L.lcm_inpaint_mask_prepare(_p(mask_u8), _p(weights_u32), int(radius), _p(alpha_out), _p(scratch), _p(latmask_out),
                                          int(B), int(H), int(W), _stream()), "lcm_inpaint_mask_prepare")
    launches = (2 if int(radius) > 0 else 0) + (1 if latmask_out is not None else 0)
    for _ in range(launches):
        _record_plain(lambda: inpaint_mask_prepare(mask_u8, weights_u32, radius, alpha_out, scratch, latmask_out, B, H, W))
    return launches


def scheduler_step_inpaint(eps, lat, noise, z, e1, latmask, coef6, last, next_sqrt_a, next_sqrt_b, B, h, w, *, eps_uncond=None,
                           guidance=1.0, pred="epsilon", dup=False):
    if pred not in _lib.PREDICTION_TYPES:
        raise ValueError(f"unknown prediction type {pred!r}: expected one of {sorted(_lib.PREDICTION_TYPES)}")
    L = _lib.load()
    arr = (C.c_float * 6)(*[float(c) for c in coef6])
    rc = L.lcm_scheduler_step_inpaint(_p(eps), _p(eps_uncond), float(guidance), _p(lat), _p(noise), _p(z), _p(e1), _p(latmask), arr,
                                      int(bool(last)), float(next_sqrt_a), float(next_sqrt_b), _lib.PREDICTION_TYPES[pred],
                                      int(B), int(h), int(w), int(bool(dup)), _stream())
    _lib.check(rc, "lcm_scheduler_step_inpaint")
    _record_plain(lambda: scheduler_step_inpaint(eps, lat, noise, z, e1, latmask, coef6, last, next_sqrt_a, next_sqrt_b, B, h, w,
                                                 eps_uncond=eps_uncond, guidance=guidance, pred=pred, dup=dup))
    return lat


def inpaint_composite_rgb8(rgb, init_u8, alpha_u8, B, H, W):
    L = _lib.load()
    _lib.check(L.lcm_inpaint_composite_rgb8(_p(rgb), _p(init_u8), _p(alpha_u8), int(B), int(H), int(W), _stream()),
               "lcm_inpaint_composite_rgb8")
    _record_plain(lambda: inpaint_composite_rgb8(rgb, init_u8, alpha_u8, B, H, W))
    return rgb


def canny_ws_bytes(B, H, W):
    return int(_lib.load().lcm_canny_ws_bytes(int(B), int(H), int(W)))


def canny_classes(rgb_u8, cls_out, B, H, W, lo, hi):
    L = _lib.load()
    _lib.check(L.lcm_canny_classes_u8(_p(rgb_u8), _p(cls_out), int(B), int(H), int(W), int(lo), int(hi), _stream()),
               "lcm_canny_classes_u8")
    return cls_out


def canny_link(cls_u8, out_rgb, ws, B, H, W):
    L = _lib.load()
    _lib.check(L.lcm_canny_link(_p(cls_u8), _p(out_rgb), _p(ws), int(ws.numel() * ws.element_size()), int(B), int(H), int(W),
                                _stream()), "lcm_canny_link")
    return out_rgb


def canny_rgb8(rgb_u8, out_rgb, ws, B, H, W, low=100.0, high=200.0):
    L = _lib.load()
    _lib.check(L.lcm_canny_rgb8(_p(rgb_u8), _p(out_rgb), _p(ws), int(ws.numel() * ws.element_size()), int(B), int(H), int(W),
                                float(low), float(high), _stream()), "lcm_canny_rgb8")
    return out_rgb


def invert_u8(x, out):
    L = _lib.load()
    _lib.check(L.lcm_invert_u8(_p(x), _p(out), int(x.numel()), _stream()), "lcm_invert_u8")
    return out


def noise_variation(lat0, B, h, w, descs):
    L = _lib.load()
    if len(descs) != int(B):
        raise ValueError(f"noise_variation: {len(descs)} descriptors for a batch of {B}")
    arr = (_lib.VariationDesc * max(int(B), 1))()
    for b, d in enumerate(descs):
        if d is None:
            continue
        low, high, hs, ws, t = d
        arr[b] = _lib.VariationDesc(_p(lat0[b]) if low is None else _p(low), _p(high), int(hs), int(ws), float(t), 1)
    _lib.check(L.lcm_noise_variation_f32(_p(lat0), int(B), int(h), int(w), arr, _stream()), "lcm_noise_variation_f32")
    return lat0


def _resize_geometry(src, out_w, out_h, window):
    if src.dtype != torch.uint8 or src.dim() not in (2, 3) or (src.dim() == 3 and src.shape[2] not in (1, 3)):
        raise _lib.LcmHipError(f"resize: the source must be uint8 [H,W], [H,W,1] or [H,W,3], got {src.dtype} {tuple(src.shape)}")
    Cn = 1 if src.dim() == 2 else int(src.shape[2])
    x0, y0, w, h = (0, 0, out_w, out_h) if window is None else window
    return Cn, int(src.shape[1]), int(src.shape[0]), int(out_w), int(out_h), int(x0), int(y0), int(w), int(h)


def resize_ws_bytes(src_w, src_h, channels, out_w, out_h, window=None):
    x0, y0, w, h = (0, 0, out_w, out_h) if window is None else window
    return int(_lib.load().lcm_resize_ws_bytes(int(channels), int(src_w), int(src_h), int(out_w), int(out_h), int(x0), int(y0),
                                               int(w), int(h)))


@functools.lru_cache(maxsize=64)
def _resize_tables(sw, sh, out_w, out_h, x0, y0, w, h):
    L = _lib.load()
    n = int(L.lcm_resize_plan_table_bytes(sw, sh, out_w, out_h, w, h))
    if n <= 0:
        raise _lib.LcmHipError(f"resize: {sw}x{sh} -> {out_w}x{out_h} window {w}x{h} is outside the resampler's domain")
    t = torch.empty(n, dtype=torch.uint8)
    if torch.cuda.is_available():
        t = t.pin_memory()
    _lib.check(L.lcm_resize_plan_tables(sw, sh, out_w, out_h, x0, y0, w, h, C.c_void_p(t.data_ptr()), n), "lcm_resize_plan_tables")
    return t


def resize_lanczos_u8(src, dst, ws, out_w, out_h, window=None):
    L = _lib.load()
    Cn, sw, sh, ow, oh, x0, y0, w, h = _resize_geometry(src, out_w, out_h, window)
    want = (h, w) if dst.dim() == 2 else (h, w, Cn)
    if dst.dtype != torch.uint8 or tuple(dst.shape) != want:
        raise _lib.LcmHipError(f"resize: the destination must be uint8 {want}, got {dst.dtype} {tuple(dst.shape)}")
    for t, name in ((src, "source"), (dst, "destination")):
        inner = (1,) if t.dim() == 2 else (t.shape[2], 1)
        if tuple(t.stride()[1:]) != inner:
            raise _lib.LcmHipError(f"resize: the {name}'s rows must be contiguous (strides {tuple(t.stride())})")
    tab = _resize_tables(sw, sh, ow, oh, x0, y0, w, h)
    nbytes = int(ws.numel() * ws.element_size())
    if nbytes < tab.numel():
        raise _lib.LcmHipError(f"resize: workspace of {nbytes} bytes is smaller than its tables ({tab.numel()})")
    ws.view(torch.uint8).reshape(-1)[:tab.numel()].copy_(tab, non_blocking=True)
    _lib.check(L.lcm_resize_lanczos_u8(_p(src), int(src.stride(0)) if sh > 1 else sw * Cn, Cn, sw, sh, ow, oh, x0, y0, w, h, _p(dst),
                                       int(dst.stride(0)) if h > 1 else w * Cn, _p(ws), nbytes, _stream()), "lcm_resize_lanczos_u8")
    return dst


def latents_pool8(lat, out, B, h, w):
    L = _lib.load()
    _lib.check(L.lcm_latents_pool8(_p(lat), _p(out), B, h, w, _stream()), "lcm_latents_pool8")
    return out


def set_workspace(t):
    L = _lib.load()
    _lib.check(L.lcm_set_workspace(_p(t), 0 if t is None else t.numel() * t.element_size()), "lcm_set_workspace")


def set_stream_workspace(stream, t, forget=False):
    L = _lib.load()
    nbytes = 0 if (t is None or forget) else t.numel() * t.element_size()
    _lib.check(L.lcm_set_stream_workspace(C.c_void_p(stream.cuda_stream), _p(t), nbytes), "lcm_set_stream_workspace")


_OWN_STREAMS = {}


def acquire_stream(device):
    import torch
    dev = torch.device(device)
    idx = dev.index if dev.index is not None else torch.cuda.current_device()
    idle = _OWN_STREAMS.setdefault(idx, [])
    if idle:
        return idle.pop()
    L = _lib.load()
    out = C.c_void_p()
    with torch.cuda.device(idx):
        _lib.check(L.lcm_stream_create(C.byref(out)), "lcm_stream_create")
    return torch.cuda.ExternalStream(out.value, device=torch.device("cuda", idx))


def release_stream(stream):
    if stream is not None:
        _OWN_STREAMS.setdefault(stream.device.index, []).append(stream)


def set_tuning(target_wgs=0, max_splits=0, min_wgs=0):
    _lib.check(_lib.load().lcm_set_tuning(int(target_wgs), int(max_splits), int(min_wgs)), "lcm_set_tuning")


def set_split_policy(max_rows_per_image=4096, max_parts=8):
    _lib.check(_lib.load().lcm_set_split_policy(int(max_rows_per_image), int(max_parts)), "lcm_set_split_policy")


def set_attention_waves(waves):
    _lib.check(_lib.load().lcm_set_attention_waves(int(waves)), "lcm_set_attention_waves")


def set_attention_impl(impl):
    _lib.check(_lib.load().lcm_set_attention_impl(int(impl)), "lcm_set_attention_impl")


def set_attention_ksplit(on):
    _lib.check(_lib.load().lcm_set_attention_ksplit(int(on)), "lcm_set_attention_ksplit")


def set_seg_mode(mode):
    _lib.check(_lib.load().lcm_set_seg_mode(int(mode)), "lcm_set_seg_mode")


def set_gn_fused_bytes(n):
    _lib.check(_lib.load().lcm_set_gn_fused_bytes(int(n)), "lcm_set_gn_fused_bytes")


def set_kernel_variant(v):
    _lib.check(_lib.load().lcm_set_kernel_variant(int(v)), "lcm_set_kernel_variant")


def profile_begin(max_launches=1 << 17):
    _lib.check(_lib.load().lcm_profile_begin(int(max_launches)), "lcm_profile_begin")


def profile_end():
    buf = C.create_string_buffer(1 << 24)
    n = _lib.load().lcm_profile_end(buf, len(buf))
    if n < 0:
        _lib.check(n, "lcm_profile_end")
    out = []
    for line in buf.value.decode().splitlines():
        name, ms = line.rsplit("\t", 1)
        out.append((name, float(ms)))
    return out


def axpy(base, delta, alpha, out):
    _lib.check(_lib.load().lcm_axpy_f16(_p(base), _p(delta), float(alpha), _p(out), base.numel(), _stream()), "lcm_axpy_f16")
    return out


def vae_blend(a, ah, aw, b, bh, bw, B, extent, vertical):
    _lib.check(_lib.load().lcm_vae_blend_f32(_p(a), ah, aw, _p(b), bh, bw, B, extent, 1 if vertical else 0, _stream()), "lcm_vae_blend_f32")


def vae_place_tile(tile, th, tw, out_u8, out_f32, H, W, B, oy, ox, ch, cw):
    _lib.check(_lib.load().lcm_vae_place_tile(_p(tile), th, tw, _p(out_u8), _p(out_f32), H, W, B, oy, ox, ch, cw, _stream()),
               "lcm_vae_place_tile")


def set_staged_epilogue(on):
    _lib.check(_lib.load().lcm_set_staged_epilogue(int(on)), "lcm_set_staged_epilogue")


def debug_spin(usec):
    _lib.check(_lib.load().lcm_debug_spin(int(usec), _stream()), "lcm_debug_spin")


class Graph:

    def __init__(self):
        self._exec = C.c_void_p()

    def __enter__(self):
        _lib.check(_lib.load().lcm_graph_begin(_stream()), "lcm_graph_begin")
        return self

    def __exit__(self, et, ev, tb):
        rc = _lib.load().lcm_graph_end(_stream(), C.byref(self._exec))
        if et is None:
            _lib.check(rc, "lcm_graph_end")
        return False

    def launch(self):
        _lib.check(_lib.load().lcm_graph_launch(self._exec, _stream()), "lcm_graph_launch")

    def close(self):
        if self._exec:
            _lib.load().lcm_graph_destroy(self._exec)
            self._exec = C.c_void_p()

    def __del__(self):
        try:
            self.close()
        except Exception:
            pass
```

Measured before the change: 52.37 images/s.

## Split wide VAE attention over key ranges and parallelize groupnorm stat finalize

Adds a split-K flash attention path for head dim 512 with 1K-4K keys, used by the VAE mid-block. It runs four key partitions in parallel with LDS-DMA double buffering and merges them in a separate combine kernel. It also adds a chunked two-stage groupnorm finalize for inputs with many stat slabs, which spreads what was a serial reduction across more blocks. In exchange it writes fp32 partial buffers and launches extra kernels.

```diff
diff --git a/include/lcm_hip.h b/include/lcm_hip.h
--- a/include/lcm_hip.h
+++ b/include/lcm_hip.h
@@ -100,6 +100,13 @@
                                  const void* stats2, int P2, const void* gamma, const void* beta, void* out,
                                  int B, int HW, int groups, float eps, int silu, void* ws, void* stream);
 
+int lcm_gn_finalize_chunks(int P, int C, int groups);
+int lcm_groupnorm_from_stats_wide_f16(const void* x, const void* stats, int P, const void* gamma, const void* beta, void* out,
+                                      int B, int HW, int C, int groups, float eps, int silu, void* tables, void* part,
+                                      int64_t part_bytes, void* stream);
+int lcm_groupnorm_tables_wide_f32(const void* stats, int P, const void* gamma, const void* beta, void* tables, int B, int HW,
+                                  int C, int groups, float eps, void* part, int64_t part_bytes, void* stream);
+
 int lcm_layernorm_f16(const void* x, const void* gamma, const void* beta, void* out, int M, int C, float eps,
                       void* stream);
 
@@ -108,6 +115,10 @@
 int lcm_set_attention_waves(int waves);
 int lcm_set_attention_impl(int impl);
 int lcm_set_attention_ksplit(int on);
+int lcm_attention_key_parts(int Sk, int d);
+int64_t lcm_attention_split_ws_bytes(int B, int heads, int Sq, int Sk, int d);
+int lcm_attention_split_f16(const void* Q, int ldq, const void* K, int ldk, const void* V, int ldv, void* out, int ldo,
+                            int B, int heads, int Sq, int Sk, int d, float scale, void* ws, int64_t ws_bytes, void* stream);
 
 int lcm_embed_tokens_f16(const void* ids, const void* tok_emb, const void* pos_emb, void* out, int B, int S, int D,
                          int vocab, void* stream);
diff --git a/stable-diffusion-1.5-lcm-onnx-rknn2_amd/csrc/attention_split.hip b/stable-diffusion-1.5-lcm-onnx-rknn2_amd/csrc/attention_split.hip
--- /dev/null
+++ b/stable-diffusion-1.5-lcm-onnx-rknn2_amd/csrc/attention_split.hip
@@ -0,0 +1,291 @@
+#include "common.h"
+#include <type_traits>
+#include <utility>
+
+extern "C" int lcm_attention_f16(const void* Q, int ldq, const void* K, int ldk, const void* V, int ldv, void* out, int ldo,
+                                 int B, int heads, int Sq, int Sk, int d, float scale, int causal, void* stream);
+
+static inline int attn_key_parts(int Sk, int d) {
+    if (d != 512 || Sk < 1024) return 1;
+    if (Sk <= 4096) return 4;
+    return 1;
+}
+static inline long long attn_split_ws_floats(int B, int heads, int Sq, int parts) {
+    return (long long)parts * B * heads * Sq * (512 + 2);
+}
+
+struct AttnSplitParams {
+    const half_t* Q; const half_t* K; const half_t* V;
+    float* Op;
+    float* ML;
+    int ldq, ldk, ldv;
+    int B, heads, Sq, Sk;
+    int parts, tpp;
+    float sc;
+};
+
+template <int N>
+__device__ __forceinline__ void asp_wait_vmcnt() {
+    asm volatile("s_waitcnt vmcnt(%0)" ::"n"(N) : "memory");
+}
+template <int... I, class F>
+__device__ __forceinline__ void asp_static_for_impl(std::integer_sequence<int, I...>, F&& f) {
+    (f(std::integral_constant<int, I>{}), ...);
+}
+template <int N, class F>
+__device__ __forceinline__ void asp_static_for(F&& f) {
+    asp_static_for_impl(std::make_integer_sequence<int, N>{}, f);
+}
+template <int OFF>
+__device__ __forceinline__ s4 asp_tr_read(unsigned lds_addr) {
+    s4 v;
+    asm volatile("ds_read_b64_tr_b16 %0, %1 offset:%2" : "=v"(v) : "v"(lds_addr), "n"(OFF));
+    return v;
+}
+
+template <int D, int TK>
+__global__ __launch_bounds__(256, 1) void attn_wide_part_kernel(AttnSplitParams p) {
+    static_assert(D == 512 && TK == 32, "one LDS-DMA instruction per 1 KB row; 8 rows of K and of V per wave per tile");
+    constexpr int RS = D * 2 + 32;
+    constexpr int NKS = D / 32, NDB = D / 16, NKB = TK / 16;
+    constexpr int TILE = TK * RS, BUF = 2 * TILE;
+    extern __shared__ __attribute__((aligned(16))) char smem[];
+
+    const int tid = threadIdx.x, lane = tid & 63, wave = tid >> 6;
+    const int frow = lane & 15, fq = lane >> 4;
+    const int qb = blockIdx.x / p.parts, part = blockIdx.x - qb * p.parts;
+    const int bh = blockIdx.y, b = bh / p.heads, head = bh - b * p.heads;
+    const int qrow = qb * 64 + wave * 16 + frow;
+    const half_t* Qb = p.Q + (long long)b * p.Sq * p.ldq + head * D;
+    const half_t* Kb = p.K + (long long)b * p.Sk * p.ldk + head * D + lane * 8;
+    const half_t* Vb = p.V + (long long)b * p.Sk * p.ldv + head * D + lane * 8;
+
+    auto issue_tile = [&](int t, int buf) {
+        char* ks = smem + buf * BUF + wave * (TK / 4) * RS;
+#pragma unroll
+        for (int i = 0; i < TK / 4; ++i) {
+            const int key = t * TK + wave * (TK / 4) + i;
+            const int kc = key < p.Sk ? key : p.Sk - 1;
+            __builtin_amdgcn_global_load_lds((const __attribute__((address_space(1))) void*)(Kb + (long long)kc * p.ldk),
+                                             (__attribute__((address_space(3))) void*)(ks + i * RS), 16, 0, 0);
+            __builtin_amdgcn_global_load_lds((const __attribute__((address_space(1))) void*)(Vb + (long long)kc * p.ldv),
+                                             (__attribute__((address_space(3))) void*)(ks + TILE + i * RS), 16, 0, 0);
+        }
+    };
+    const int ntiles = (p.Sk + TK - 1) / TK;
+    const int t0 = part * p.tpp, t1 = min(t0 + p.tpp, ntiles);
+    if (t0 < t1) issue_tile(t0, 0);
+
+    h8 qf[NKS];
+#pragma unroll
+    for (int ks = 0; ks < NKS; ++ks) {
+        h8 v = {0, 0, 0, 0, 0, 0, 0, 0};
+        if (qrow < p.Sq) v = *reinterpret_cast<const h8*>(Qb + (long long)qrow * p.ldq + 32 * ks + 8 * fq);
+        qf[ks] = v;
+    }
+    f4 oacc[NDB];
+#pragma unroll
+    for (int i = 0; i < NDB; ++i) oacc[i] = (f4){0.f, 0.f, 0.f, 0.f};
+    float m_run = -1.0e30f, l_run = 0.f;
+
+    const int k_addr = frow * RS + fq * 16;
+    const int v_addr = TILE + (4 * fq + (frow >> 2)) * RS + (4 * (frow & 3)) * 2;
+    for (int t = t0; t < t1; ++t) {
+        const int buf = (t - t0) & 1;
+        asp_wait_vmcnt<0>();
+        __builtin_amdgcn_s_barrier();
+        if (t + 1 < t1) issue_tile(t + 1, buf ^ 1);
+        const char* Ks = smem + buf * BUF;
+
+        f4 sacc[NKB];
+#pragma unroll
+        for (int kb = 0; kb < NKB; ++kb) sacc[kb] = (f4){0.f, 0.f, 0.f, 0.f};
+        {
+            constexpr int G = 8 / NKB, NG = NKS / G;
+            h8 kfr[2][8];
+            auto rd = [&](int g, h8* dst) {
+#pragma unroll
+                for (int kb = 0; kb < NKB; ++kb)
+#pragma unroll
+                    for (int j = 0; j < G; ++j)
+                        dst[kb * G + j] = *reinterpret_cast<const h8*>(Ks + k_addr + kb * 16 * RS + (g * G + j) * 64);
+            };
+            rd(0, kfr[0]);
+#pragma unroll
+            for (int g = 0; g < NG; ++g) {
+                if (g + 1 < NG) rd(g + 1, kfr[(g + 1) & 1]);
+                __builtin_amdgcn_sched_barrier(0);
+#pragma unroll
+                for (int j = 0; j < G; ++j)
+#pragma unroll
+                    for (int kb = 0; kb < NKB; ++kb)
+                        sacc[kb] = __builtin_amdgcn_mfma_f32_16x16x32_f16(kfr[g & 1][kb * G + j], qf[g * G + j], sacc[kb], 0, 0, 0);
+                __builtin_amdgcn_sched_barrier(0);
+            }
+        }
+        if (t == ntiles - 1 && (p.Sk % TK)) {
+#pragma unroll
+            for (int kb = 0; kb < NKB; ++kb)
+#pragma unroll
+                for (int j = 0; j < 4; ++j)
+                    if (t * TK + kb * 16 + 4 * fq + j >= p.Sk) sacc[kb][j] = -1.0e30f;
+        }
+        float mt = -1.0e30f;
+#pragma unroll
+        for (int kb = 0; kb < NKB; ++kb)
+#pragma unroll
+            for (int j = 0; j < 4; ++j) mt = fmaxf(mt, sacc[kb][j]);
+        mt = fmaxf(mt, __shfl_xor(mt, 16, 64));
+        mt = fmaxf(mt, __shfl_xor(mt, 32, 64));
+        const float m_new = fmaxf(m_run, mt * p.sc);
+        if (!__all(m_new == m_run)) {
+            const float alpha = __builtin_amdgcn_exp2f(m_run - m_new);
+            l_run *= alpha;
+#pragma unroll
+            for (int i = 0; i < NDB; ++i) { oacc[i][0] *= alpha; oacc[i][1] *= alpha; oacc[i][2] *= alpha; oacc[i][3] *= alpha; }
+            m_run = m_new;
+        }
+        h8 pf[NKB / 2];
+#pragma unroll
+        for (int kb = 0; kb < NKB; ++kb)
+#pragma unroll
+            for (int j = 0; j < 4; ++j) {
+                const float pv = __builtin_amdgcn_exp2f(sacc[kb][j] * p.sc - m_run);
+                l_run += pv;
+                pf[kb >> 1][(kb & 1) * 4 + j] = (half_t)pv;
+            }
+        {
+            static_assert(NKB == 2, "one key pair per tile");
+            constexpr int GD = 4, NG = NDB / GD;
+            s4 vfr[2][2 * GD];
+            const unsigned vbase = (unsigned)(size_t)(__attribute__((address_space(3))) const char*)(Ks + v_addr);
+            asp_static_for<GD>([&](auto j) {
+                constexpr int J = decltype(j)::value;
+                vfr[0][2 * J] = asp_tr_read<J * 32>(vbase);
+                vfr[0][2 * J + 1] = asp_tr_read<J * 32 + 16 * RS>(vbase);
+            });
+            asp_static_for<NG>([&](auto g) {
+                constexpr int Gi = decltype(g)::value;
+                s4* cur = vfr[Gi & 1];
+                if constexpr (Gi + 1 < NG) {
+                    s4* nxt = vfr[(Gi + 1) & 1];
+                    asp_static_for<GD>([&](auto j) {
+                        constexpr int J = decltype(j)::value;
+                        nxt[2 * J] = asp_tr_read<((Gi + 1) * GD + J) * 32>(vbase);
+                        nxt[2 * J + 1] = asp_tr_read<((Gi + 1) * GD + J) * 32 + 16 * RS>(vbase);
+                    });
+                    asm volatile("s_waitcnt lgkmcnt(8)" : "+v"(cur[0]), "+v"(cur[1]), "+v"(cur[2]), "+v"(cur[3]),
+                                 "+v"(cur[4]), "+v"(cur[5]), "+v"(cur[6]), "+v"(cur[7]));
+                } else {
+                    asm volatile("s_waitcnt lgkmcnt(0)" : "+v"(cur[0]), "+v"(cur[1]), "+v"(cur[2]), "+v"(cur[3]),
+                                 "+v"(cur[4]), "+v"(cur[5]), "+v"(cur[6]), "+v"(cur[7]));
+                }
+                __builtin_amdgcn_sched_barrier(0);
+#pragma unroll
+                for (int j = 0; j < GD; ++j) {
+                    const h4 lo_h = __builtin_bit_cast(h4, cur[2 * j]), hi_h = __builtin_bit_cast(h4, cur[2 * j + 1]);
+                    const h8 vf = {lo_h[0], lo_h[1], lo_h[2], lo_h[3], hi_h[0], hi_h[1], hi_h[2], hi_h[3]};
+                    oacc[Gi * GD + j] = __builtin_amdgcn_mfma_f32_16x16x32_f16(vf, pf[0], oacc[Gi * GD + j], 0, 0, 0);
+                }
+                __builtin_amdgcn_sched_barrier(0);
+            });
+        }
+    }
+    float l_tot = l_run + __shfl_xor(l_run, 16, 64);
+    l_tot += __shfl_xor(l_tot, 32, 64);
+    if (qrow < p.Sq) {
+        const long long R = (long long)p.B * p.heads * p.Sq;
+        const long long r = (long long)part * R + (long long)bh * p.Sq + qrow;
+        float* orow = p.Op + r * D;
+#pragma unroll
+        for (int db = 0; db < NDB; ++db) *reinterpret_cast<f4*>(orow + db * 16 + 4 * fq) = oacc[db];
+        if (fq == 0) *reinterpret_cast<float2*>(p.ML + r * 2) = make_float2(m_run, l_tot);
+    }
+}
+
+template <int D, int PARTS>
+__global__ __launch_bounds__(256) void attn_wide_combine_kernel(const float* __restrict__ Op, const float* __restrict__ ML,
+                                                                half_t* __restrict__ O, int ldo, long long R, int Sq, int heads) {
+    static_assert(D == 512, "128 threads x 4 channels");
+    const long long r = (long long)blockIdx.x * 2 + (threadIdx.x >> 7);
+    if (r >= R) return;
+    const int j = threadIdx.x & 127;
+    float2 ml[PARTS];
+    f4 o[PARTS];
+#pragma unroll
+    for (int q = 0; q < PARTS; ++q) {
+        ml[q] = *reinterpret_cast<const float2*>(ML + ((long long)q * R + r) * 2);
+        o[q] = *reinterpret_cast<const f4*>(Op + ((long long)q * R + r) * D + 4 * j);
+    }
+    float M = ml[0].x;
+#pragma unroll
+    for (int q = 1; q < PARTS; ++q) M = fmaxf(M, ml[q].x);
+    float L = 0.f;
+    f4 acc = {0.f, 0.f, 0.f, 0.f};
+#pragma unroll
+    for (int q = 0; q < PARTS; ++q) {
+        const float w = __builtin_amdgcn_exp2f(ml[q].x - M);
+        L = __builtin_fmaf(w, ml[q].y, L);
+#pragma unroll
+        for (int i = 0; i < 4; ++i) acc[i] = __builtin_fmaf(w, o[q][i], acc[i]);
+    }
+    const float inv = 1.0f / L;
+    const long long bh = r / Sq;
+    const int q_ = (int)(r - bh * Sq);
+    const long long b = bh / heads;
+    const int head = (int)(bh - b * heads);
+    const h4 out = {(half_t)(acc[0] * inv), (half_t)(acc[1] * inv), (half_t)(acc[2] * inv), (half_t)(acc[3] * inv)};
+    *reinterpret_cast<h4*>(O + (b * Sq + q_) * ldo + head * D + 4 * j) = out;
+}
+
+template <int PARTS>
+static void launch_combine(const AttnSplitParams& p, half_t* out, int ldo, hipStream_t s) {
+    const long long R = (long long)p.B * p.heads * p.Sq;
+    hipLaunchKernelGGL((attn_wide_combine_kernel<512, PARTS>), dim3((unsigned)((R + 1) / 2)), dim3(256), 0, s, p.Op, p.ML, out, ldo,
+                       R, p.Sq, p.heads);
+}
+
+extern "C" int lcm_attention_key_parts(int Sk, int d) { return attn_key_parts(Sk, d); }
+
+extern "C" int64_t lcm_attention_split_ws_bytes(int B, int heads, int Sq, int Sk, int d) {
+    const int parts = attn_key_parts(Sk, d);
+    if (parts <= 1 || B <= 0 || heads <= 0 || Sq <= 0) return 0;
+    return attn_split_ws_floats(B, heads, Sq, parts) * 4;
+}
+
+extern "C" int lcm_attention_split_f16(const void* Q, int ldq, const void* K, int ldk, const void* V, int ldv, void* out,
+                                       int ldo, int B, int heads, int Sq, int Sk, int d, float scale, void* ws,
+                                       int64_t ws_bytes, void* stream) {
+    const int parts = attn_key_parts(Sk, d);
+    if (parts <= 1)
+        return lcm_attention_f16(Q, ldq, K, ldk, V, ldv, out, ldo, B, heads, Sq, Sk, d, scale, 0, stream);
+    LCM_REQUIRE(parts == 4, "attention_split: no combine kernel for %d key ranges", parts);
+    LCM_REQUIRE(Q && K && V && out && ws, "attention_split: null pointer");
+    LCM_REQUIRE(B > 0 && heads > 0 && Sq > 0, "attention_split: bad shape");
+    LCM_REQUIRE(ldq % 8 == 0 && ldk % 8 == 0 && ldv % 8 == 0 && ldo % 4 == 0, "attention_split: misaligned leading dims");
+    LCM_REQUIRE(((uintptr_t)ws & 15) == 0, "attention_split: partial buffer not 16-byte aligned");
+    const long long need = attn_split_ws_floats(B, heads, Sq, parts) * 4;
+    LCM_REQUIRE(ws_bytes >= need, "attention_split: partial buffer too small (%lld bytes, need %lld)", (long long)ws_bytes, need);
+    constexpr int TK = 32;
+    const int ntiles = (Sk + TK - 1) / TK, tpp = (ntiles + parts - 1) / parts;
+    LCM_REQUIRE((parts - 1) * tpp < ntiles, "attention_split: empty key range");
+    const long long R = (long long)B * heads * Sq;
+    const long long nqb = (Sq + 63) / 64;
+    LCM_REQUIRE(nqb * parts < (1ll << 31) && (long long)B * heads <= 65535, "attention_split: grid too large");
+    AttnSplitParams p = {(const half_t*)Q, (const half_t*)K, (const half_t*)V, (float*)ws, (float*)ws + (long long)parts * R * 512,
+                         ldq, ldk, ldv, B, heads, Sq, Sk, parts, tpp,
+                         scale > 0.f ? scale * 1.4426950408889634f : 1.0f};
+    hipStream_t s = (hipStream_t)stream;
+    constexpr int LDS = 2 * 2 * TK * (512 * 2 + 32);
+    static LcmDevOnce attr_once;
+    if (auto once_guard = attr_once.first()) {
+        once_guard.check(hipFuncSetAttribute(reinterpret_cast<const void*>(&attn_wide_part_kernel<512, TK>), hipFuncAttributeMaxDynamicSharedMemorySize, LDS));
+    }
+    lcm_prof_start("attn_wide_part_kernel<512,32>", s);
+    hipLaunchKernelGGL((attn_wide_part_kernel<512, TK>), dim3((unsigned)(nqb * parts), B * heads), dim3(256), LDS, s, p);
+    lcm_prof_stop(s);
+    LCM_CHECK_LAUNCH("attention_wide_part");
+    launch_combine<4>(p, (half_t*)out, ldo, s);
+    LCM_CHECK_LAUNCH("attention_wide_combine");
+    return LCM_OK;
+}
diff --git a/stable-diffusion-1.5-lcm-onnx-rknn2_amd/csrc/gn_finalize_wide.hip b/stable-diffusion-1.5-lcm-onnx-rknn2_amd/csrc/gn_finalize_wide.hip
--- /dev/null
+++ b/stable-diffusion-1.5-lcm-onnx-rknn2_amd/csrc/gn_finalize_wide.hip
@@ -0,0 +1,149 @@
+#include "common.h"
+
+#define GNW_MIN_SLABS 2048
+#define GNW_LD 8
+
+static inline int gn_wide_spc(int P) {
+    int s = P / 256;
+    if (s < 8) s = 8;
+    if (s > 32) s = 32;
+    return s;
+}
+static inline bool gn_wide_serves(int P, int C, int groups) {
+    return P >= GNW_MIN_SLABS && groups > 0 && groups <= 64 && (C == 64 || C == 128 || C == 256 || C == 512) && C % groups == 0;
+}
+static inline int gn_wide_chunks(int P) { const int s = gn_wide_spc(P); return (P + s - 1) / s; }
+
+__global__ __launch_bounds__(256) void gn_slab_chunk_kernel(const float* __restrict__ st, int P, int C, int spc, int groups,
+                                                            float* __restrict__ part) {
+    __shared__ float sm_s[512], sm_q[512];
+    const int tid = threadIdx.x, chunk = blockIdx.x, b = blockIdx.y, nchunk = gridDim.x;
+    const int p0 = chunk * spc, nslab = min(spc, P - p0);
+    const int per = nslab * C;
+    const float2* base = reinterpret_cast<const float2*>(st) + ((long long)b * P + p0) * C;
+    const bool two = C > 256;
+    float s0 = 0.f, q0 = 0.f, s1 = 0.f, q1 = 0.f;
+    for (int i0 = tid; i0 < per; i0 += 256 * GNW_LD) {
+        float2 v[GNW_LD];
+#pragma unroll
+        for (int k = 0; k < GNW_LD; ++k) v[k] = base[min(i0 + 256 * k, per - 1)];
+#pragma unroll
+        for (int k = 0; k < GNW_LD; ++k) {
+            const bool in = i0 + 256 * k < per;
+            const float ax = in ? v[k].x : 0.f, ay = in ? v[k].y : 0.f;
+            if (two && (k & 1)) { s1 = in ? s1 + ax : s1; q1 = in ? q1 + ay : q1; }
+            else { s0 = in ? s0 + ax : s0; q0 = in ? q0 + ay : q0; }
+        }
+    }
+    sm_s[tid] = s0; sm_q[tid] = q0;
+    sm_s[256 + tid] = s1; sm_q[256 + tid] = q1;
+    __syncthreads();
+    if (tid < groups) {
+        const int cpg = C / groups;
+        const int span = two ? 512 : 256, rl_n = span / C;
+        float s = 0.f, q = 0.f;
+        for (int rl = 0; rl < rl_n; ++rl)
+            for (int j = 0; j < cpg; ++j) {
+                const int idx = rl * C + tid * cpg + j;
+                s += sm_s[idx]; q += sm_q[idx];
+            }
+        float* o = part + (((long long)b * nchunk + chunk) * groups + tid) * 2;
+        o[0] = s; o[1] = q;
+    }
+}
+
+__global__ __launch_bounds__(64) void gn_fold_chunks_kernel(const float* __restrict__ part, const half_t* __restrict__ gamma,
+                                                            const half_t* __restrict__ beta, float* __restrict__ scale,
+                                                            float* __restrict__ shift, int nchunk, int groups, int C,
+                                                            float inv_count, float eps) {
+    const int bg = blockIdx.x, b = bg / groups, g = bg - b * groups, lane = threadIdx.x;
+    float s = 0.f, q = 0.f;
+    for (int c = lane; c < nchunk; c += 64) {
+        const float* p = part + (((long long)b * nchunk + c) * groups + g) * 2;
+        s += p[0]; q += p[1];
+    }
+    s = wave_sum(s); q = wave_sum(q);
+    const float mean = s * inv_count;
+    const float rstd = rsqrtf(fmaxf(q * inv_count - mean * mean, 0.f) + eps);
+    const int cpg = C / groups;
+    for (int j = lane; j < cpg; j += 64) {
+        const int c = g * cpg + j;
+        const float a = rstd * (float)gamma[c];
+        scale[(long long)b * C + c] = a;
+        shift[(long long)b * C + c] = (float)beta[c] - mean * a;
+    }
+}
+
+__global__ __launch_bounds__(256) void gn_apply1_kernel(const half_t* __restrict__ x, const float* __restrict__ scale,
+                                                        const float* __restrict__ shift, half_t* __restrict__ out, int HW, int C,
+                                                        int silu, int rows_per_wg) {
+    const int ncc = C >> 3, nrl = 256 / ncc;
+    const int b = blockIdx.y, tid = threadIdx.x;
+    const int rl = tid / ncc, c = (tid - rl * ncc) * 8;
+    const int r0 = blockIdx.x * rows_per_wg, r1 = min(HW, r0 + rows_per_wg);
+    const long long rowbase = (long long)b * HW;
+    float sc[8], sh[8];
+#pragma unroll
+    for (int j = 0; j < 8; ++j) { sc[j] = scale[(long long)b * C + c + j]; sh[j] = shift[(long long)b * C + c + j]; }
+    auto one = [&](h8 v) {
+        h8 o;
+#pragma unroll
+        for (int j = 0; j < 8; ++j) {
+            float f = __builtin_fmaf((float)v[j], sc[j], sh[j]);
+            if (silu) f = silu_f(f);
+            o[j] = (half_t)f;
+        }
+        return o;
+    };
+    int r = r0 + rl;
+    for (; r + nrl < r1; r += 2 * nrl) {
+        const h8 v0 = *reinterpret_cast<const h8*>(x + (rowbase + r) * C + c);
+        const h8 v1 = *reinterpret_cast<const h8*>(x + (rowbase + r + nrl) * C + c);
+        *reinterpret_cast<h8*>(out + (rowbase + r) * C + c) = one(v0);
+        *reinterpret_cast<h8*>(out + (rowbase + r + nrl) * C + c) = one(v1);
+    }
+    for (; r < r1; r += nrl) *reinterpret_cast<h8*>(out + (rowbase + r) * C + c) = one(*reinterpret_cast<const h8*>(x + (rowbase + r) * C + c));
+}
+
+extern "C" int lcm_gn_finalize_chunks(int P, int C, int groups) {
+    return gn_wide_serves(P, C, groups) ? gn_wide_chunks(P) : 0;
+}
+
+extern "C" int lcm_groupnorm_tables_wide_f32(const void* stats, int P, const void* gamma, const void* beta, void* tables, int B,
+                                             int HW, int C, int groups, float eps, void* part, int64_t part_bytes, void* stream) {
+    LCM_REQUIRE(stats && gamma && beta && tables && part, "groupnorm_tables_wide: null pointer");
+    LCM_REQUIRE(B > 0 && B <= 65535 && HW > 0, "groupnorm_tables_wide: bad shape");
+    LCM_REQUIRE(gn_wide_serves(P, C, groups), "groupnorm_tables_wide: P=%d C=%d groups=%d is not served (P >= %d, C in 64/128/256/512)",
+                P, C, groups, GNW_MIN_SLABS);
+    const int nchunk = gn_wide_chunks(P);
+    const long long need = (long long)B * nchunk * groups * 2 * 4;
+    LCM_REQUIRE(part_bytes >= need, "groupnorm_tables_wide: partial buffer too small (%lld bytes, need %lld)", (long long)part_bytes, need);
+    LCM_REQUIRE(((uintptr_t)stats & 7) == 0, "groupnorm_tables_wide: statistics not 8-byte aligned");
+    hipStream_t s = (hipStream_t)stream;
+    hipLaunchKernelGGL(gn_slab_chunk_kernel, dim3(nchunk, B), dim3(256), 0, s, (const float*)stats, P, C, gn_wide_spc(P), groups,
+                       (float*)part);
+    LCM_CHECK_LAUNCH("gn_slab_chunk");
+    float* scale = (float*)tables;
+    hipLaunchKernelGGL(gn_fold_chunks_kernel, dim3(B * groups), dim3(64), 0, s, (const float*)part, (const half_t*)gamma,
+                       (const half_t*)beta, scale, scale + (long long)B * C, nchunk, groups, C,
+                       1.0f / ((float)HW * (float)(C / groups)), eps);
+    LCM_CHECK_LAUNCH("gn_fold_chunks");
+    return LCM_OK;
+}
+
+extern "C" int lcm_groupnorm_from_stats_wide_f16(const void* x, const void* stats, int P, const void* gamma, const void* beta,
+                                                 void* out, int B, int HW, int C, int groups, float eps, int silu, void* tables,
+                                                 void* part, int64_t part_bytes, void* stream) {
+    LCM_REQUIRE(x && out, "groupnorm_from_stats_wide: null pointer");
+    int rc = lcm_groupnorm_tables_wide_f32(stats, P, gamma, beta, tables, B, HW, C, groups, eps, part, part_bytes, stream);
+    if (rc) return rc;
+    const int nrl = 256 / (C >> 3);
+    long long rows = ((long long)B * HW + 1023) / 1024;
+    if (rows < nrl) rows = nrl;
+    if (rows > 16ll * nrl) rows = 16ll * nrl;
+    const float* scale = (const float*)tables;
+    hipLaunchKernelGGL(gn_apply1_kernel, dim3((unsigned)((HW + rows - 1) / rows), B), dim3(256), 0, (hipStream_t)stream,
+                       (const half_t*)x, scale, scale + (long long)B * C, (half_t*)out, HW, C, silu, (int)rows);
+    LCM_CHECK_LAUNCH("gn_apply1");
+    return LCM_OK;
+}
diff --git a/stable-diffusion-1.5-lcm-onnx-rknn2_amd/lib.py b/stable-diffusion-1.5-lcm-onnx-rknn2_amd/lib.py
--- a/stable-diffusion-1.5-lcm-onnx-rknn2_amd/lib.py
+++ b/stable-diffusion-1.5-lcm-onnx-rknn2_amd/lib.py
@@ -38,6 +38,9 @@
     "lcm_ln_fold_refresh": [_vp, _i, _i, _vp, _vp, _f, _vp, _vp, _vp],
     "lcm_conv3x3_f16": [_vp, _vp, _vp, _vp, _i, _vp, _vp, _i, _i, _i, _i, _i, _i, _i, _vp, _i64, C.POINTER(_i), _vp],
     "lcm_groupnorm_from_stats_f16": [_vp, _i, _vp, _i, _vp, _i, _vp, _i, _vp, _vp, _vp, _i, _i, _i, _f, _i, _vp, _vp],
+    "lcm_groupnorm_tables_wide_f32": [_vp, _i, _vp, _vp, _vp, _i, _i, _i, _i, _f, _vp, _i64, _vp],
+    "lcm_gn_finalize_chunks": [_i, _i, _i],
+    "lcm_groupnorm_from_stats_wide_f16": [_vp, _vp, _i, _vp, _vp, _vp, _i, _i, _i, _i, _f, _i, _vp, _vp, _i64, _vp],
     "lcm_conv3x3_c4_f32in": [_vp, _vp, _vp, _f, _vp, _vp, _vp, _i, _i, _i, _i, _vp],
     "lcm_conv3x3_c4_res_f32in": [_vp, _vp, _vp, _vp, _vp, _i, _i, _i, _i, _vp],
     "lcm_hint_conv_u8": [_vp, _vp, _vp, _vp, _i, _i, _i, _i, _i, _vp],
@@ -47,6 +50,8 @@
     "lcm_groupnorm_f16": [_vp, _i, _vp, _i, _vp, _vp, _vp, _i, _i, _i, _f, _i, _vp, _vp],
     "lcm_layernorm_f16": [_vp, _vp, _vp, _vp, _i, _i, _f, _vp],
     "lcm_attention_f16": [_vp, _i, _vp, _i, _vp, _i, _vp, _i, _i, _i, _i, _i, _i, _f, _i, _vp],
+    "lcm_attention_split_f16": [_vp, _i, _vp, _i, _vp, _i, _vp, _i, _i, _i, _i, _i, _i, _f, _vp, _i64, _vp],
+    "lcm_attention_key_parts": [_i, _i],
     "lcm_embed_tokens_f16": [_vp, _vp, _vp, _vp, _i, _i, _i, _i, _vp],
     "lcm_prompt_emphasis_f16": [_vp, _vp, _vp, _i, _i, _i, _i, _vp],
     "lcm_softmax_rows_f16": [_vp, _i, _i, _i, _vp],
@@ -130,7 +135,7 @@
 }
 EXPORTS = tuple(sorted(list(_SIGS) + ["lcm_last_error", "lcm_version", "lcm_groupnorm_ws_bytes", "lcm_stats_bytes", "lcm_png_bound",
                               "lcm_canny_ws_bytes", "lcm_jpeg_coef_bytes", "lcm_jpeg_bound", "lcm_resize_ws_bytes",
-                              "lcm_resize_table_bytes", "lcm_resize_plan_table_bytes"]))
+                              "lcm_resize_table_bytes", "lcm_resize_plan_table_bytes", "lcm_attention_split_ws_bytes"]))
 
 EUNSUPPORTED = -3
 
@@ -166,6 +171,8 @@
     lib.lcm_png_bound.restype = C.c_longlong
     lib.lcm_png_bound.argtypes = [_i, _i, _i]
     lib.lcm_stats_bytes.argtypes = [_i, _i, _i]
+    lib.lcm_attention_split_ws_bytes.restype = _i64
+    lib.lcm_attention_split_ws_bytes.argtypes = [_i] * 5
     lib.lcm_canny_ws_bytes.restype = C.c_longlong
     lib.lcm_canny_ws_bytes.argtypes = [_i, _i, _i]
     for fn, n in ((lib.lcm_resize_ws_bytes, 9), (lib.lcm_resize_table_bytes, 3), (lib.lcm_resize_plan_table_bytes, 6)):
diff --git a/stable-diffusion-1.5-lcm-onnx-rknn2_amd/model.py b/stable-diffusion-1.5-lcm-onnx-rknn2_amd/model.py
--- a/stable-diffusion-1.5-lcm-onnx-rknn2_amd/model.py
+++ b/stable-diffusion-1.5-lcm-onnx-rknn2_amd/model.py
@@ -70,7 +70,8 @@
         C = C1 + C2
         ws = self.gn_ws(B, HW, C)
         if x_st is not None and x_st.P > 0 and (x2 is None or (x2_st is not None and x2_st.P > 0)):
-            ops.groupnorm_from_stats(x, gamma, beta, out, B, HW, C1, x_st, ws, x2=x2, C2=C2, st2=x2_st, eps=eps, silu=silu)
+            ops.groupnorm_from_stats(x, gamma, beta, out, B, HW, C1, x_st, ws, x2=x2, C2=C2, st2=x2_st, eps=eps, silu=silu,
+                                     scratch=self.gn_scratch(B, x_st, C1) if x2 is None else None)
         else:
             ops.groupnorm(x, gamma, beta, out, B, HW, C1, ws, x2=x2, C2=C2, eps=eps, silu=silu)
         return out
@@ -78,7 +79,8 @@
     def _norm_conv_out(self, x, norm, st, hn, out, B, H, W, ch, cout, eps, *, mode, out_f32=None):
         wt = self.w
         if st is not None and st.P > 0 and ch % 64 == 0:
-            sc_t, sh_t = ops.groupnorm_tables_from_stats(wt[norm + ".g"], wt[norm + ".b"], B, H * W, ch, st, self.gn_ws(B, H * W, ch), eps=eps)
+            sc_t, sh_t = ops.groupnorm_tables_from_stats(wt[norm + ".g"], wt[norm + ".b"], B, H * W, ch, st, self.gn_ws(B, H * W, ch), eps=eps,
+                                                         scratch=self.gn_scratch(B, st, ch))
             ops.conv3x3_smalln(x, wt["conv_out.w"], out, B, H, W, ch, cout, bias=wt["conv_out.b"], mode=mode, out_f32=out_f32,
                                gn_scale=sc_t, gn_shift=sh_t, silu=True)
         else:
@@ -90,6 +92,17 @@
         t = self._stats.get(key)
         if t is None:
             t = torch.empty(max(ops.groupnorm_ws_bytes(B, HW, C) // 4, 1024), dtype=torch.float32, device=self.device)
+            self._stats[key] = t
+        return t
+
+    def gn_scratch(self, B, st, C):
+        n = ops.gn_finalize_scratch_floats(B, st.P, C)
+        if not n:
+            return None
+        key = ("gn_parts", n)
+        t = self._stats.get(key)
+        if t is None:
+            t = ops.GnScratch(torch.empty(n, dtype=torch.float32, device=self.device))
             self._stats[key] = t
         return t
 
@@ -121,7 +134,8 @@
         h1_st = self.stats("conv1", M, Cout, HW)
         if have1 and C1 % 64 == 0 and C2 % 64 == 0 and _fuse_gn_into_conv(M, Cin, Cout):
             sc_t, sh_t = ops.groupnorm_tables_from_stats(w[p + ".norm1.g"], w[p + ".norm1.b"], B, HW, C1, x_st, self.gn_ws(B, HW, Cin),
-                                                         C2=C2, st2=x2_st if x2 is not None else None, eps=eps)
+                                                         C2=C2, st2=x2_st if x2 is not None else None, eps=eps,
+                                                         scratch=self.gn_scratch(B, x_st, C1) if x2 is None else None)
             ops.conv3x3_gn(x, w[p + ".conv1.w"], h1, B, H, W, C1, Cout, x2=x2, C2=C2, gn_scale=sc_t, gn_shift=sh_t, silu=True,
                            bias=w[p + ".conv1.b"], rowadd=rowadd, stats=h1_st)
         else:
@@ -132,7 +146,7 @@
         out_st = self.stats(out_role, M, Cout, HW)
         if h1_st.P > 0 and _fuse_gn_into_conv(M, Cout, Cout):
             sc_t, sh_t = ops.groupnorm_tables_from_stats(w[p + ".norm2.g"], w[p + ".norm2.b"], B, HW, Cout, h1_st,
-                                                         self.gn_ws(B, HW, Cout), eps=eps)
+                                                         self.gn_ws(B, HW, Cout), eps=eps, scratch=self.gn_scratch(B, h1_st, Cout))
             ops.conv3x3_gn(h1, w[p + ".conv2.w"], out, B, H, W, Cout, Cout, gn_scale=sc_t, gn_shift=sh_t, silu=True,
                            bias=w[p + ".conv2.b"], res=sc, stats=out_st)
         else:
@@ -583,7 +597,10 @@
             qkv = self.buf.get("attn_qkv", M, 3 * C)
             ops.gemm(hn, w["attn.qkv.w"], qkv, bias=w["attn.qkv.b"], img_rows=S)
             o = self.buf.get("attn_o", M, C)
-            ops.attention(qkv[:, :C], qkv[:, C:2 * C], qkv[:, 2 * C:], o, B, 1, S, S, C, ldq=3 * C, ldk=3 * C, ldv=3 * C, ldo=C)
+            nws = ops.attention_scratch_floats(B, 1, S, S, C)
+            ws = ops.AttnScratch(self.buf.get("attn_parts", nws, dtype=torch.float32)) if nws else None
+            ops.attention(qkv[:, :C], qkv[:, C:2 * C], qkv[:, 2 * C:], o, B, 1, S, S, C, ldq=3 * C, ldk=3 * C, ldv=3 * C, ldo=C,
+                          scratch=ws)
             ops.gemm(o, w["attn.o.w"], out, bias=w["attn.o.b"], res=x, stats=out_st, img_rows=S)
             return out, out_st
         Sp = -(-S // 64) * 64
@@ -789,7 +806,8 @@
         pre_m = self.buf.get("pre_mean", B, H, W, 4, dtype=torch.float32)
         pre_l = self.buf.get("pre_logvar", B, H, W, 4, dtype=torch.float32)
         if st is not None and st.P > 0 and ch % 64 == 0:
-            sc_t, sh_t = ops.groupnorm_tables_from_stats(wt["norm_out.g"], wt["norm_out.b"], B, H * W, ch, st, self.gn_ws(B, H * W, ch), eps=1e-6)
+            sc_t, sh_t = ops.groupnorm_tables_from_stats(wt["norm_out.g"], wt["norm_out.b"], B, H * W, ch, st, self.gn_ws(B, H * W, ch), eps=1e-6,
+                                                         scratch=self.gn_scratch(B, st, ch))
             for n, o in (("mean", pre_m), ("logvar", pre_l)):
                 ops.conv3x3_smalln(x, wt[f"conv_out.{n}.w"], o, B, H, W, ch, 4, bias=wt[f"conv_out.{n}.b"], mode=0,
                                    gn_scale=sc_t, gn_shift=sh_t, silu=True)
diff --git a/stable-diffusion-1.5-lcm-onnx-rknn2_amd/ops.py b/stable-diffusion-1.5-lcm-onnx-rknn2_amd/ops.py
--- a/stable-diffusion-1.5-lcm-onnx-rknn2_amd/ops.py
+++ b/stable-diffusion-1.5-lcm-onnx-rknn2_amd/ops.py
@@ -345,8 +345,17 @@
     return out
 
 
-def groupnorm_from_stats(x, gamma, beta, out, B, HW, C1, st1, ws, *, x2=None, C2=0, st2=None, groups=32, eps=1e-5, silu=True):
-    L = _lib.load()
+def groupnorm_from_stats(x, gamma, beta, out, B, HW, C1, st1, ws, *, x2=None, C2=0, st2=None, groups=32, eps=1e-5, silu=True,
+                         scratch=None):
+    L = _lib.load()
+    if x2 is None and st2 is None and gn_finalize_chunks(st1.P, C1, groups):
+        need = gn_finalize_scratch_floats(B, st1.P, C1, groups)
+        part = scratch.buf if scratch is not None else torch.empty(need, dtype=torch.float32, device=ws.device)
+        rc = L.lcm_groupnorm_from_stats_wide_f16(_p(x), _p(st1.buf), st1.P, _p(gamma), _p(beta), _p(out), B, HW, C1, groups,
+                                                 float(eps), 1 if silu else 0, _p(ws), _p(part),
+                                                 part.numel() * part.element_size(), _stream())
+        _lib.check(rc, "lcm_groupnorm_from_stats_wide_f16")
+        return out
     rc = L.lcm_groupnorm_from_stats_f16(_p(x), C1, _p(x2), C2 if x2 is not None else 0, _p(st1.buf), st1.P,
                                         _p(st2.buf) if st2 is not None else None, st2.P if st2 is not None else 0,
                                         _p(gamma), _p(beta), _p(out), B, HW, groups, float(eps), 1 if silu else 0, _p(ws), _stream())
@@ -354,9 +363,36 @@
     return out
 
 
-def groupnorm_tables_from_stats(gamma, beta, B, HW, C1, st1, ws, *, C2=0, st2=None, groups=32, eps=1e-5):
+@functools.lru_cache(maxsize=None)
+def gn_finalize_chunks(P, C, groups=32):
+    return int(_lib.load().lcm_gn_finalize_chunks(int(P), int(C), int(groups)))
+
+
+def gn_finalize_scratch_floats(B, P, C, groups=32):
+    return 2 * B * gn_finalize_chunks(P, C, groups) * groups
+
+
+class GnScratch:
+
+    __slots__ = ("buf",)
+
+    def __init__(self, buf):
+        self.buf = buf
+
+    def __repr__(self):
+        return f"GnScratch({self.buf.numel()})"
+
+
+def groupnorm_tables_from_stats(gamma, beta, B, HW, C1, st1, ws, *, C2=0, st2=None, groups=32, eps=1e-5, scratch=None):
     L = _lib.load()
     C = C1 + (C2 if st2 is not None else 0)
+    if st2 is None and gn_finalize_chunks(st1.P, C1, groups):
+        need = gn_finalize_scratch_floats(B, st1.P, C1, groups)
+        part = scratch.buf if scratch is not None else torch.empty(need, dtype=torch.float32, device=ws.device)
+        rc = L.lcm_groupnorm_tables_wide_f32(_p(st1.buf), st1.P, _p(gamma), _p(beta), _p(ws), B, HW, C1, groups, float(eps),
+                                             _p(part), part.numel() * part.element_size(), _stream())
+        _lib.check(rc, "lcm_groupnorm_tables_wide_f32")
+        return ws[:B * C].view(B, C), ws[B * C:2 * B * C].view(B, C)
     rc = L.lcm_groupnorm_from_stats_f16(None, C1, None, C2 if st2 is not None else 0, _p(st1.buf), st1.P,
                                         _p(st2.buf) if st2 is not None else None, st2.P if st2 is not None else 0,
                                         _p(gamma), _p(beta), None, B, HW, groups, float(eps), 0, _p(ws), _stream())
@@ -386,13 +422,43 @@
     return out
 
 
-def attention(q, k, v, out, B, heads, Sq, Sk, d, *, ldq, ldk, ldv, ldo, scale=None, causal=False):
+@functools.lru_cache(maxsize=None)
+def attention_key_parts(Sk, d, causal=False):
+    return 1 if causal else int(_lib.load().lcm_attention_key_parts(int(Sk), int(d)))
+
+
+def attention_scratch_floats(B, heads, Sq, Sk, d, causal=False):
+    if attention_key_parts(Sk, d, causal) == 1:
+        return 0
+    return int(_lib.load().lcm_attention_split_ws_bytes(int(B), int(heads), int(Sq), int(Sk), int(d))) // 4
+
+
+class AttnScratch:
+
+    __slots__ = ("buf",)
+
+    def __init__(self, buf):
+        self.buf = buf
+
+    def __repr__(self):
+        return f"AttnScratch({self.buf.numel()})"
+
+
+def attention(q, k, v, out, B, heads, Sq, Sk, d, *, ldq, ldk, ldv, ldo, scale=None, causal=False, scratch=None):
     L = _lib.load()
     scale = d ** -0.5 if scale is None else scale
     RECORD = _record_list()
     if RECORD is not None:
         RECORD.append((None, None, lambda: attention(q, k, v, out, B, heads, Sq, Sk, d, ldq=ldq, ldk=ldk, ldv=ldv, ldo=ldo,
-                                                     scale=scale, causal=causal)))
+                                                     scale=scale, causal=causal, scratch=scratch)))
+    need = attention_scratch_floats(B, heads, Sq, Sk, d, causal)
+    if need:
+        ws = scratch.buf if scratch is not None else torch.empty(need, dtype=torch.float32, device=out.device)
+        with _Timed("attention", 4.0 * B * heads * Sq * Sk * d, 2.0 * B * heads * d * (2 * Sq + 2 * Sk)):
+            rc = L.lcm_attention_split_f16(_p(q), ldq, _p(k), ldk, _p(v), ldv, _p(out), ldo, B, heads, Sq, Sk, d, float(scale),
+                                           _p(ws), ws.numel() * ws.element_size(), _stream())
+        _lib.check(rc, "lcm_attention_split_f16")
+        return out
     with _Timed("attention", 4.0 * B * heads * Sq * Sk * d, 2.0 * B * heads * d * (2 * Sq + 2 * Sk)):
         rc = L.lcm_attention_f16(_p(q), ldq, _p(k), ldk, _p(v), ldv, _p(out), ldo, B, heads, Sq, Sk, d, float(scale),
                                  1 if causal else 0, _stream())
```

Result: no change. 52.89 images/s (median of 6 runs) (+1.0%).
